# NVlabs/UnseenObjectClustering

Hardware: AMD Instinct MI355X
Metric: frames/sec at 640x480 RGB-D, two-stage clustering (higher is better)
Workload: dtype f32; 1 GPU; configs[3] frames: full two-stage (crop-and-refine) segmentation of single 640x480 RGB-D frames; throughput schedule 3 streams x 4-frame launch sets (one frame at a time: `latency`); frame=640x480, seeds=100, iters=10, crop=224, total_frames=513, frames_per_gpu=513, collective=False, frames_in_flight_per_gpu=12, streams_per_gpu=3, frames_per_launch=4

## Files before the change

include/uoc_hip.h:

```cpp
#ifndef UOC_HIP_H
#define UOC_HIP_H

#include <stddef.h>
#include <stdint.h>

#ifdef __cplusplus
extern "C" {
#endif

#define UOC_OK 0
#define UOC_EINVAL (-22)
#define UOC_ENOMEM (-12)
#define UOC_EHIP (-5)
#define UOC_ENOENT (-2)
#define UOC_ETIMEDOUT (-110)

#define UOC_EMBED_DIM 64
#define UOC_MAX_SEEDS 128
#define UOC_METRIC_COSINE 0
#define UOC_METRIC_EUCLIDEAN 1

int uoc_version(void);
int uoc_is_dev_build(void);
unsigned long long uoc_config_fingerprint(void);
int uoc_shutdown(void);
const char *uoc_last_error(void);
int uoc_reload_env(void);


int uoc_ms_set_persistent_fps(int on);
int uoc_ms_set_stream_ordering(int on);
int uoc_ms_fps_fallbacks(void);
int uoc_ms_check(void *stream);

size_t uoc_ms_workspace_bytes(int batch, int n, int m);

int uoc_ms_select_seeds(const float *d_X, int batch, int n, int m, const int32_t *d_first_index,
                        float *d_seeds, int32_t *d_indices, void *d_ws, size_t ws_bytes, void *stream);

int uoc_ms_select_seeds_from(const float *d_X, int batch, int n, int m, int num_init, const int32_t *d_first_index,
                             float *d_seeds, int32_t *d_indices, void *d_ws, size_t ws_bytes, void *stream);

int uoc_ms_hill_climb(const float *d_X, int batch, int n, float *d_Z, int m, float kappa, int iters,
                      void *d_ws, size_t ws_bytes, void *stream);

int uoc_ms_seed_components(const float *d_Z, int batch, int m, float epsilon, int32_t *d_seed_labels,
                           int32_t *d_num_unique, void *stream);

int uoc_ms_assign(const float *d_X, int batch, int n, const float *d_Z, const int32_t *d_seed_labels,
                  const int32_t *d_num_unique, int m, int32_t *d_labels, int32_t *d_closest,
                  void *d_ws, size_t ws_bytes, void *stream);

int uoc_ms_cluster(const float *d_X, int batch, int n, int m, float kappa, int iters, float epsilon,
                   const int32_t *d_first_index, int32_t *d_labels, int32_t *d_indices,
                   float *d_Z_out, int32_t *d_seed_labels_out, void *d_ws, size_t ws_bytes, void *stream);

size_t uoc_ms_workspace_bytes_wide(int batch, int n, int m, int halves);
int uoc_ms_cluster_wide(const float *d_X, int halves, int batch, int n, int m, float kappa, int iters, float epsilon,
                        const int32_t *d_first_index, int32_t *d_labels, int32_t *d_indices, float *d_Z_out,
                        int32_t *d_seed_labels_out, void *d_ws, size_t ws_bytes, void *stream);

int uoc_ms_select_seeds_ex(const float *d_X, int batch, int n, int m, int num_init, const int32_t *d_first_index,
                           float *d_seeds, int32_t *d_indices, int metric, void *d_ws, size_t ws_bytes, void *stream);
int uoc_ms_hill_climb_ex(const float *d_X, int batch, int n, float *d_Z, int m, float kappa, int iters, int metric,
                         void *d_ws, size_t ws_bytes, void *stream);
int uoc_ms_seed_components_ex(const float *d_Z, int batch, int m, float epsilon, int metric, int32_t *d_seed_labels,
                              int32_t *d_num_unique, void *stream);
int uoc_ms_assign_ex(const float *d_X, int batch, int n, const float *d_Z, const int32_t *d_seed_labels,
                     const int32_t *d_num_unique, int m, int metric, int32_t *d_labels, int32_t *d_closest, void *d_ws,
                     size_t ws_bytes, void *stream);
int uoc_ms_cluster_ex(const float *d_X, int batch, int n, int m, float kappa, int iters, float epsilon, int metric,
                      const int32_t *d_first_index, int32_t *d_labels, int32_t *d_indices, float *d_Z_out,
                      int32_t *d_seed_labels_out, void *d_ws, size_t ws_bytes, void *stream);
int uoc_ms_cluster_wide_ex(const float *d_X, int halves, int batch, int n, int m, float kappa, int iters, float epsilon,
                           int metric, const int32_t *d_first_index, int32_t *d_labels, int32_t *d_indices, float *d_Z_out,
                           int32_t *d_seed_labels_out, void *d_ws, size_t ws_bytes, void *stream);


typedef struct uoc_net uoc_net;

enum { UOC_NET_RGBD_ADD = 0, UOC_NET_COLOR = 1, UOC_NET_DEPTH = 2, UOC_NET_RGBD_EARLY = 3, UOC_NET_RGBD_CAT = 4 };

int uoc_net_create(uoc_net **out);
int uoc_net_create_mode(uoc_net **out, int mode);
int uoc_net_embed_dim(const uoc_net *net);
int uoc_net_destroy(uoc_net *net);
int uoc_net_load_param(uoc_net *net, const char *name, const float *host_data, size_t numel);
int uoc_net_finalize(uoc_net *net);
size_t uoc_net_workspace_bytes(const uoc_net *net, int B, int H, int W);
int uoc_net_set_split_precision(uoc_net *net, int on);
int uoc_net_forward(uoc_net *net, const float *d_rgb, const float *d_xyz, int B, int H, int W, float *d_embed,
                    void *d_ws, size_t ws_bytes, void *stream);

#define UOC_CONV_DIRECT 0
#define UOC_CONV_WINOGRAD4 4
#define UOC_CONV_WINOGRAD4_BF16X3 5
int uoc_conv2d_nhwc(const float *d_in, const float *d_w, const float *d_bias, const float *d_res, float *d_out,
                    int G, int B, int H, int W, int Cin, int Cout, int K, int stride, int dil, int pad, int relu,
                    void *stream);
int uoc_conv2d_nhwc_algo(const float *d_in, const float *d_w, const float *d_bias, const float *d_res, float *d_out,
                         int G, int B, int H, int W, int Cin, int Cout, int K, int stride, int dil, int pad, int relu,
                         int algo, void *stream);

int uoc_conv2d_tile_list(int algo, int32_t *out_pairs, int cap);
int uoc_conv2d_nhwc_tile(const float *d_in, const float *d_w, const float *d_bias, const float *d_res, float *d_out,
                         int G, int B, int H, int W, int Cin, int Cout, int K, int stride, int dil, int pad, int relu,
                         int algo, void *stream, int cfg, int bm);
int uoc_conv2d_tile_choice(int G, int B, int H, int W, int Cin, int Cout, int K, int stride, int dil, int algo,
                           int32_t *cfg, int32_t *bm, int32_t *family_bm);
int uoc_net_stem(const float *d_nchw, const float *h_w, const float *h_bias, const float *d_res, int G, int B, int H,
                 int W, int relu, float *d_out, void *stream);
int uoc_maxpool3x3s2_nhwc(const float *d_in, float *d_out, int n_img, int H, int W, int C, void *stream);
int uoc_head(const float *d_fa, const float *d_fb, float *d_embed, int B, int h, int w, int H, int W, int cat,
             void *stream);


typedef struct uoc_roi_table {
  int32_t K;
  int32_t label[128];
  int32_t box[128][4];
} uoc_roi_table;

size_t uoc_roi_workspace_bytes(void);

int uoc_prep_rgbd(const uint8_t *d_bgr, const uint16_t *d_depth_mm, int H, int W, float fx, float fy, float px,
                  float py, float mean_b, float mean_g, float mean_r, float *d_image, float *d_xyz, void *stream);

int uoc_filter_labels_depth(int32_t *d_labels, const float *d_z, long z_batch_stride, int B, int H, int W,
                            float threshold, void *d_ws, size_t ws_bytes, void *stream);

int uoc_roi_build(int32_t *d_labels, const float *d_z, int H, int W, float threshold, float pad_fraction,
                  uoc_roi_table *d_table, void *d_ws, size_t ws_bytes, void *stream);

int uoc_roi_crop(const float *d_rgb, const float *d_xyz, const int32_t *d_labels, int H, int W,
                 const uoc_roi_table *d_table, int K, int S, float *d_rgb_crops, float *d_xyz_crops,
                 float *d_mask_crops, void *stream);

int uoc_roi_match_stats(const int32_t *d_labels_crop, const float *d_mask_crops, const float *d_xyz_crops, int K,
                        int S, int32_t *d_keep, float *d_meanz, void *d_ws, size_t ws_bytes, void *stream);

int uoc_roi_paste(const int32_t *d_labels_crop, const uoc_roi_table *d_table, const int32_t *d_map,
                  const int32_t *d_order, int K, int S, int H, int W, int32_t *d_refined, void *stream);

int uoc_roi_match(const int32_t *d_labels_crop, const float *d_mask_crops, const float *d_xyz_crops,
                  const uoc_roi_table *d_table, int K, int S, int H, int W, int32_t *d_refined, int32_t *d_keep,
                  int32_t *d_plan, int32_t *d_status, void *d_ws, size_t ws_bytes, void *stream);

int uoc_labels_to_u8(const int32_t *d_labels, long n, uint8_t *d_out, int32_t *d_top, void *stream);


typedef struct uoc_eval_tables {
  int32_t cont[128 * 128];
  int32_t prec_tp[128 * 128];
  int32_t rec_tp[128 * 128];
  int32_t bnd_pred[128];
  int32_t bnd_gt[128];
  int32_t bad_label;
} uoc_eval_tables;

size_t uoc_eval_workspace_bytes(int H, int W);
int uoc_eval_pair_stats(const int32_t *d_pred, const int32_t *d_gt, int H, int W, int radius, uoc_eval_tables *d_tables,
                        void *d_ws, size_t ws_bytes, void *stream);


#define UOC_OBJECTS_MAX_ATTR 8
typedef struct uoc_object {
  int32_t pixels;
  int32_t count;
  int32_t box[4];
  float centroid[3];
  float cov[6];
  float aabb_min[3];
  float aabb_max[3];
  float eig[3];
  float axes[9];
  float obb_center[3];
  float obb_half[3];
  int32_t offset;
  int32_t kept;
} uoc_object;

size_t uoc_objects_workspace_bytes(int B, int H, int W);
int uoc_objects(const int32_t *d_labels, const float *d_xyz, const float *d_attr, int attr_ch, int B, int H, int W,
                int max_points_per_object, uoc_object *d_objects, float *d_points, float *d_point_attr,
                int32_t *d_point_pixel, long capacity, int32_t *d_total, void *d_ws, size_t ws_bytes, void *stream);


typedef struct uoc_track {
  int32_t uid;
  int32_t age;
  int32_t hits;
  int32_t area;
  int32_t born;
} uoc_track;
#define UOC_TRACK_SLOTS 128
#define UOC_TRACK_HEADER_WORDS 1024
#define UOC_TRACK_META_WORD 640
#define UOC_TRACK_CONT_WORDS (128 * 128)

size_t uoc_track_state_bytes(int B, int H, int W);
size_t uoc_track_workspace_bytes(int B);
int uoc_track_reset(void *d_state, int B, int H, int W, int which, void *stream);
int uoc_track_step(const int32_t *d_labels, int B, int H, int W, int q, int max_age, void *d_state, int32_t *d_out,
                   int32_t *d_lut, uoc_track *d_tracks, void *d_ws, size_t ws_bytes, void *stream);


#define UOC_CC_ALL 0
#define UOC_CC_LARGEST 1

size_t uoc_cc_workspace_bytes(int B, int H, int W);
int uoc_cc_split(const int32_t *d_labels, int B, int H, int W, int connectivity, int min_area, int mode, int32_t *d_out,
                 int32_t *d_table, int32_t *d_counts, void *d_ws, size_t ws_bytes, void *stream);


typedef struct uoc_plane {
  int32_t found;
  int32_t candidates;
  int32_t inliers;
  int32_t hyp;
  float normal[3];
  float d;
  float centroid[3];
  float eig[3];
  float rms;
  float u[3];
  float v[3];
} uoc_plane;

typedef struct uoc_plane_object {
  int32_t count;
  float height_min;
  float height_max;
  float foot[2];
  float cov2[3];
  float axis[2];
  float half[3];
  float center[3];
} uoc_plane_object;
#define UOC_PLANE_MAX_HYP 1024
#define UOC_PLANE_MAX_TAU_MM 1000

size_t uoc_plane_workspace_bytes(int B, int H, int W, int num_hyp);
int uoc_support_plane(const int32_t *d_labels, const float *d_xyz, int B, int H, int W, int num_hyp, int tau_mm,
                      uint32_t seed, uoc_plane *d_planes, uoc_plane_object *d_objs, float *d_height, void *d_ws,
                      size_t ws_bytes, void *stream);


typedef struct uoc_plane_info {
  int32_t round_candidates;
  int32_t removed;
  float cos0;
  float offset0;
  float extent[4];
} uoc_plane_info;
#define UOC_PLANES_MAX 8
#define UOC_PLANES_FRINGE 16

size_t uoc_planes_workspace_bytes(int B, int H, int W, int num_hyp, int max_planes);
int uoc_support_planes(const int32_t *d_labels, const float *d_xyz, int B, int H, int W, int max_planes, int num_hyp,
                       int tau_mm, int rem_mm, int min_inliers, uint32_t seed, int32_t *d_count, uoc_plane *d_planes,
                       uoc_plane_info *d_info, int32_t *d_index, uoc_plane_object *d_objs, void *d_ws, size_t ws_bytes,
                       void *stream);


#define UOC_REL_BORDER 0
#define UOC_REL_TOUCH 1
#define UOC_REL_FRONT 2
#define UOC_REL_MAX_GAP_MM 65535

typedef struct uoc_relation_object {
  int32_t pixels;
  int32_t edge;
  int32_t border;
  int32_t border_bg;
  int32_t hidden;
  int32_t n_touch;
  int32_t n_above;
  int32_t n_below;
  int32_t layer;
  int32_t free;
  int32_t order;
} uoc_relation_object;

size_t uoc_relations_workspace_bytes(int B, int H, int W);
int uoc_relations(const int32_t *d_labels, const float *d_xyz, int B, int H, int W, int connectivity, int gap_mm,
                  int min_pairs, int32_t *d_pairs, uoc_relation_object *d_objs, void *d_ws, size_t ws_bytes, void *stream);


#define UOC_PLACE_MAX_QUERIES 16
#define UOC_PLACE_WIDEST 0
#define UOC_PLACE_NEAREST 1
#define UOC_PLACE_MAX_GRID 512
#define UOC_PLACE_MAX_MM 1000
#define UOC_PLACE_MAX_MIN_PTS 65535
#define UOC_PLACE_MAX_ANCHOR 4096
#define UOC_PLACE_SCALE 16384

size_t uoc_placement_workspace_bytes(int B, int H, int W, int G);
int uoc_placement(const int32_t *d_labels, const float *d_xyz, const uoc_plane *d_planes, int B, int H, int W, int G,
                  int cell_mm, int h_obs_mm, int tau_mm, int min_pts, int unknown_blocks, const int32_t *h_queries, int Q,
                  int32_t *d_state, int32_t *d_owner, int32_t *d_dist2, int32_t *d_counts, int64_t *d_frame,
                  int32_t *d_answers, void *d_ws, size_t ws_bytes, void *stream);


#define UOC_GRASP_MAX_DIRS 32
#define UOC_GRASP_MISS (-1)
#define UOC_GRASP_WIDE (-2)
#define UOC_GRASP_PINCHED (-3)
#define UOC_GRASP_BLOCKED (-4)
#define UOC_GRASP_SCALE 16384
#define UOC_GRASP_MAX_OFFSETS 8
#define UOC_GRASP_MAX_OPEN 64
#define UOC_GRASP_MAX_GAP 4
#define UOC_GRASP_MAX_FINGER 8
#define UOC_GRASP_MAX_PAD 4

size_t uoc_grasp_workspace_bytes(int B, int G, int A, int M);
int uoc_grasp(const int32_t *d_state, const int32_t *d_owner, int B, int G, const int32_t *h_dirs, int A, int M, int Wmax,
              int gap, int F, int Hp, int unknown_blocks, int32_t *d_cand, int32_t *d_best, void *d_ws, size_t ws_bytes,
              void *stream);


#define UOC_ELEV_MAX_QUERIES 16
#define UOC_ELEV_NONE (-32768)

size_t uoc_elevation_workspace_bytes(int B, int H, int W, int G);
int uoc_elevation(const int32_t *d_labels, const float *d_xyz, const int64_t *d_frame, int B, int H, int W, int G,
                  int cell_mm, int tau_mm, int step_mm, int min_pts, const int32_t *h_queries, int Q, int32_t *d_elev,
                  int32_t *d_owner, int32_t *d_pts, int32_t *d_near, int32_t *d_dist2, int32_t *d_tops, int32_t *d_info,
                  int32_t *d_answers, void *d_ws, size_t ws_bytes, void *stream);


#define UOC_FOOT_MAX_RECTS 8
#define UOC_FOOT_MAX_HALF 16384
#define UOC_FOOT_ROOMIEST 0
#define UOC_FOOT_NEAREST 1

size_t uoc_footprint_workspace_bytes(int B, int G, int A, int F);
int uoc_footprint(const int32_t *d_state, const int32_t *d_owner, const int32_t *d_dist2, const int64_t *d_frame, int B, int G,
                  const int32_t *h_dirs, int A, const int32_t *h_rects, int F, int unknown_blocks, int32_t *d_fits,
                  int32_t *d_count, int32_t *d_best, void *d_ws, size_t ws_bytes, void *stream);


#define UOC_ROUTES_MAX_QUERIES 8
#define UOC_ROUTES_MAX_NEED2 4096
#define UOC_ROUTES_MAX_PATH 4096

size_t uoc_routes_workspace_bytes(int B, int G, int Q);
int uoc_routes(const int32_t *d_state, const int32_t *d_owner, const int64_t *d_frame, int B, int G, const int32_t *h_queries,
               int Q, int unknown_blocks, int max_path, int32_t *d_cost, int32_t *d_info, int32_t *d_path, void *d_ws,
               size_t ws_bytes, void *stream);


#define UOC_CONF_MAX_N (1 << 30)
#define UOC_CONF_ONE 65536

size_t uoc_ms_confidence_workspace_bytes(int batch, int n, int m, int halves);
int uoc_ms_confidence(const float *d_X, int halves, int batch, int n, const float *d_Z, const int32_t *d_seed_labels,
                      const int32_t *d_num_unique, int m, int metric, int32_t *d_labels, float *d_margin,
                      int32_t *d_second, int32_t *d_closest, int32_t *d_rival, void *d_ws, size_t ws_bytes, void *stream);
int uoc_conf_paste(const float *d_values_crop, const int32_t *d_labels_crop, const uoc_roi_table *d_table,
                   const int32_t *d_plan, int K, int S, int H, int W, float *d_out, void *stream);
int uoc_conf_objects(const int32_t *d_labels, const float *d_conf, int B, int H, int W, int weak_q, int64_t *d_stats,
                     void *stream);


#define UOC_NORMAL_UP 1
#define UOC_NORMAL_SIDE 2
#define UOC_NORMAL_OBLIQUE 3
#define UOC_NORMAL_DOWN 4
#define UOC_NORMALS_MAX_DIRS 32
#define UOC_NORMALS_FACE_WORDS 40

size_t uoc_normals_workspace_bytes(int B, int H, int W);
int uoc_normals(const float *d_xyz, const int32_t *d_labels, const uoc_plane *d_planes, int B, int H, int W, int step,
                int window, int jump_mm, int min_pairs, const int32_t *h_dirs, int A, int c_up, int s_side, int32_t *d_n,
                float *d_unit, int32_t *d_faces, void *d_ws, size_t ws_bytes, void *stream);


#define UOC_SIG_WORDS 104
#define UOC_SIG_MAX_N (1 << 24)
#define UOC_SIG_PIXELS 0
#define UOC_SIG_VALID 1
#define UOC_SIG_AREA 2
#define UOC_SIG_HIST 8
#define UOC_SIG_DARK 89
#define UOC_SIG_INTENSITY 90
#define UOC_IDENT_WORDS 5
#define UOC_IDENT_HEADER_WORDS 1024
#define UOC_IDENT_META_WORD 640

size_t uoc_signature_workspace_bytes(int B);
int uoc_signature(const int32_t *d_labels, const uint8_t *d_image, const float *d_xyz, int B, int H, int W, int32_t *d_sig,
                  void *d_ws, size_t ws_bytes, void *stream);
int uoc_sig_similarity(const int32_t *d_sig_a, const int32_t *d_sig_b, int B, int32_t *d_sim, void *stream);
size_t uoc_ident_state_bytes(int B);
size_t uoc_ident_workspace_bytes(int B);
int uoc_ident_reset(void *d_state, int B, int which, void *stream);
int uoc_ident_step(const int32_t *d_tracked, const uoc_track *d_tracks, const int32_t *d_sig, int B, int H, int W, int q, int r,
                   int max_lost, void *d_state, int32_t *d_out, int32_t *d_lut, int32_t *d_ident, void *d_ws, size_t ws_bytes,
                   void *stream);

#define UOC_MOTION_MAX_ROT 64
#define UOC_MOTION_MAX_RADIUS 16
#define UOC_MOTION_MAX_PAIRS 16
#define UOC_MOTION_MAX_CELLS 4096
#define UOC_MOTION_SCALE 16384
#define UOC_MOTION_ROT_WORDS 4
#define UOC_MOTION_BEST_WORDS 16

size_t uoc_motion_workspace_bytes(int B, int G, int A, int P);
int uoc_motion(const int32_t *d_state_a, const int32_t *d_owner_a, const int64_t *d_frame_a, const int32_t *d_state_b,
               const int32_t *d_owner_b, const int64_t *d_frame_b, int B, int G, const int32_t *h_rot, int A, int R,
               const int32_t *h_pairs, int P, int32_t *d_rot, int32_t *d_best, void *d_ws, size_t ws_bytes, void *stream);

#define UOC_SCENE_META_WORD 32
#define UOC_SCENE_MEM_WORD 48
#define UOC_SCENE_MAX_AGE 32767
#define UOC_SCENE_ID_WORDS 8
#define UOC_SCENE_INFO_WORDS 8
#define UOC_SCENE_SAME 0
#define UOC_SCENE_APPEARED 1
#define UOC_SCENE_VANISHED 2
#define UOC_SCENE_REOWNED 3

size_t uoc_scene_state_bytes(int B, int G);
size_t uoc_scene_workspace_bytes(int B, int G);
int uoc_scene_reset(void *d_state, int B, int G, int which, void *stream);
int uoc_scene_step(const int32_t *d_state_cur, const int32_t *d_owner_cur, const int64_t *d_frame, const int32_t *d_drop,
                   int B, int G, int max_age, int unknown_blocks, const int32_t *h_queries, int Q, void *d_mem,
                   int32_t *d_state, int32_t *d_owner, int32_t *d_dist2, int32_t *d_age, int32_t *d_change,
                   int32_t *d_ids, int32_t *d_info, int32_t *d_answers, void *d_ws, size_t ws_bytes, void *stream);


long uoc_lzf_decompress(const uint8_t *in, size_t in_len, uint8_t *out, size_t out_cap);

int uoc_prof_enable(int on);
int uoc_prof_reset(void);
int uoc_prof_report(char *buf, size_t cap);

#ifdef __cplusplus
static_assert(sizeof(uoc_roi_table) == 2564, "uoc_roi_table");
static_assert(sizeof(uoc_object) == 164, "uoc_object");
static_assert(sizeof(uoc_track) == 20, "uoc_track");
static_assert(sizeof(uoc_plane) == 84, "uoc_plane");
static_assert(sizeof(uoc_plane_object) == 64, "uoc_plane_object");
static_assert(sizeof(uoc_plane_info) == 32, "uoc_plane_info");
static_assert(sizeof(uoc_relation_object) == 44, "uoc_relation_object");
#endif

#ifdef __cplusplus
}
#endif
#endif
```

unseenobjectclustering_amd/_native.py:

```python
from __future__ import annotations

import ctypes
import os
from ctypes import c_char_p, c_float, c_int, c_int32, c_long, c_size_t, c_uint32, c_ulonglong, c_void_p, POINTER

from .build import LIB_PATH

_lib = None


class NativeError(RuntimeError):
    pass


P, I, F, Z, L, U = c_void_p, c_int, c_float, c_size_t, c_long, c_uint32
ABI = {
    "uoc_version": (I, []),
    "uoc_is_dev_build": (I, []),
    "uoc_config_fingerprint": (c_ulonglong, []),
    "uoc_shutdown": (I, []),
    "uoc_last_error": (c_char_p, []),
    "uoc_reload_env": (I, []),
    "uoc_ms_set_persistent_fps": (I, [I]),
    "uoc_ms_set_stream_ordering": (I, [I]),
    "uoc_ms_fps_fallbacks": (I, []),
    "uoc_ms_check": (I, [P]),
    "uoc_ms_workspace_bytes": (Z, [I, I, I]),
    "uoc_ms_select_seeds": (I, [P, I, I, I, P, P, P, P, Z, P]),
    "uoc_ms_select_seeds_from": (I, [P, I, I, I, I, P, P, P, P, Z, P]),
    "uoc_ms_hill_climb": (I, [P, I, I, P, I, F, I, P, Z, P]),
    "uoc_ms_seed_components": (I, [P, I, I, F, P, P, P]),
    "uoc_ms_assign": (I, [P, I, I, P, P, P, I, P, P, P, Z, P]),
    "uoc_ms_cluster": (I, [P, I, I, I, F, I, F, P, P, P, P, P, P, Z, P]),
    "uoc_ms_workspace_bytes_wide": (Z, [I, I, I, I]),
    "uoc_ms_cluster_wide": (I, [P, I, I, I, I, F, I, F, P, P, P, P, P, P, Z, P]),
    "uoc_ms_select_seeds_ex": (I, [P, I, I, I, I, P, P, P, I, P, Z, P]),
    "uoc_ms_hill_climb_ex": (I, [P, I, I, P, I, F, I, I, P, Z, P]),
    "uoc_ms_seed_components_ex": (I, [P, I, I, F, I, P, P, P]),
    "uoc_ms_assign_ex": (I, [P, I, I, P, P, P, I, I, P, P, P, Z, P]),
    "uoc_ms_cluster_ex": (I, [P, I, I, I, F, I, F, I, P, P, P, P, P, P, Z, P]),
    "uoc_ms_cluster_wide_ex": (I, [P, I, I, I, I, F, I, F, I, P, P, P, P, P, P, Z, P]),
    "uoc_net_create": (I, [POINTER(P)]),
    "uoc_net_create_mode": (I, [POINTER(P), I]),
    "uoc_net_embed_dim": (I, [P]),
    "uoc_net_destroy": (I, [P]),
    "uoc_net_load_param": (I, [P, c_char_p, P, Z]),
    "uoc_net_finalize": (I, [P]),
    "uoc_net_workspace_bytes": (Z, [P, I, I, I]),
    "uoc_net_set_split_precision": (I, [P, I]),
    "uoc_net_forward": (I, [P, P, P, I, I, I, P, P, Z, P]),
    "uoc_conv2d_nhwc": (I, [P, P, P, P, P, I, I, I, I, I, I, I, I, I, I, I, P]),
    "uoc_conv2d_nhwc_algo": (I, [P, P, P, P, P, I, I, I, I, I, I, I, I, I, I, I, I, P]),
    "uoc_conv2d_tile_list": (I, [I, P, I]),
    "uoc_conv2d_nhwc_tile": (I, [P, P, P, P, P, I, I, I, I, I, I, I, I, I, I, I, I, P, I, I]),
    "uoc_conv2d_tile_choice": (I, [I, I, I, I, I, I, I, I, I, I, P, P, P]),
    "uoc_net_stem": (I, [P, P, P, P, I, I, I, I, I, P, P]),
    "uoc_maxpool3x3s2_nhwc": (I, [P, P, I, I, I, I, P]),
    "uoc_head": (I, [P, P, P, I, I, I, I, I, I, P]),
    "uoc_roi_workspace_bytes": (Z, []),
    "uoc_prep_rgbd": (I, [P, P, I, I, F, F, F, F, F, F, F, P, P, P]),
    "uoc_filter_labels_depth": (I, [P, P, L, I, I, I, F, P, Z, P]),
    "uoc_roi_build": (I, [P, P, I, I, F, F, P, P, Z, P]),
    "uoc_roi_crop": (I, [P, P, P, I, I, P, I, I, P, P, P, P]),
    "uoc_roi_match_stats": (I, [P, P, P, I, I, P, P, P, Z, P]),
    "uoc_roi_paste": (I, [P, P, P, P, I, I, I, I, P, P]),
    "uoc_roi_match": (I, [P, P, P, P, I, I, I, I, P, P, P, P, P, Z, P]),
    "uoc_labels_to_u8": (I, [P, L, P, P, P]),
    "uoc_eval_workspace_bytes": (Z, [I, I]),
    "uoc_eval_pair_stats": (I, [P, P, I, I, I, P, P, Z, P]),
    "uoc_objects_workspace_bytes": (Z, [I, I, I]),
    "uoc_objects": (I, [P, P, P, I, I, I, I, I, P, P, P, P, L, P, P, Z, P]),
    "uoc_track_state_bytes": (Z, [I, I, I]),
    "uoc_track_workspace_bytes": (Z, [I]),
    "uoc_track_reset": (I, [P, I, I, I, I, P]),
    "uoc_track_step": (I, [P, I, I, I, I, I, P, P, P, P, P, Z, P]),
    "uoc_cc_workspace_bytes": (Z, [I, I, I]),
    "uoc_cc_split": (I, [P, I, I, I, I, I, I, P, P, P, P, Z, P]),
    "uoc_plane_workspace_bytes": (Z, [I, I, I, I]),
    "uoc_support_plane": (I, [P, P, I, I, I, I, I, U, P, P, P, P, Z, P]),
    "uoc_planes_workspace_bytes": (Z, [I, I, I, I, I]),
    "uoc_support_planes": (I, [P, P, I, I, I, I, I, I, I, I, U, P, P, P, P, P, P, Z, P]),
    "uoc_relations_workspace_bytes": (Z, [I, I, I]),
    "uoc_relations": (I, [P, P, I, I, I, I, I, I, P, P, P, Z, P]),
    "uoc_placement_workspace_bytes": (Z, [I, I, I, I]),
    "uoc_placement": (I, [P, P, P, I, I, I, I, I, I, I, I, I, P, I, P, P, P, P, P, P, P, Z, P]),
    "uoc_grasp_workspace_bytes": (Z, [I, I, I, I]),
    "uoc_grasp": (I, [P, P, I, I, P, I, I, I, I, I, I, I, P, P, P, Z, P]),
    "uoc_elevation_workspace_bytes": (Z, [I, I, I, I]),
    "uoc_elevation": (I, [P, P, P, I, I, I, I, I, I, I, I, P, I, P, P, P, P, P, P, P, P, P, Z, P]),
    "uoc_footprint_workspace_bytes": (Z, [I, I, I, I]),
    "uoc_footprint": (I, [P, P, P, P, I, I, P, I, P, I, I, P, P, P, P, Z, P]),
    "uoc_routes_workspace_bytes": (Z, [I, I, I]),
    "uoc_routes": (I, [P, P, P, I, I, P, I, I, I, P, P, P, P, Z, P]),
    "uoc_ms_confidence_workspace_bytes": (Z, [I, I, I, I]),
    "uoc_ms_confidence": (I, [P, I, I, I, P, P, P, I, I, P, P, P, P, P, P, Z, P]),
    "uoc_conf_paste": (I, [P, P, P, P, I, I, I, I, P, P]),
    "uoc_conf_objects": (I, [P, P, I, I, I, I, P, P]),
    "uoc_normals_workspace_bytes": (Z, [I, I, I]),
    "uoc_normals": (I, [P, P, P, I, I, I, I, I, I, I, P, I, I, I, P, P, P, P, Z, P]),
    "uoc_signature_workspace_bytes": (Z, [I]),
    "uoc_signature": (I, [P, P, P, I, I, I, P, P, Z, P]),
    "uoc_sig_similarity": (I, [P, P, I, P, P]),
    "uoc_ident_state_bytes": (Z, [I]),
    "uoc_ident_workspace_bytes": (Z, [I]),
    "uoc_ident_reset": (I, [P, I, I, P]),
    "uoc_ident_step": (I, [P, P, P, I, I, I, I, I, I, P, P, P, P, P, Z, P]),
    "uoc_motion_workspace_bytes": (Z, [I, I, I, I]),
    "uoc_motion": (I, [P, P, P, P, P, P, I, I, P, I, I, P, I, P, P, P, Z, P]),
    "uoc_scene_state_bytes": (Z, [I, I]),
    "uoc_scene_workspace_bytes": (Z, [I, I]),
    "uoc_scene_reset": (I, [P, I, I, I, P]),
    "uoc_scene_step": (I, [P, P, P, P, I, I, I, I, P, I, P, P, P, P, P, P, P, P, P, P, Z, P]),
    "uoc_lzf_decompress": (L, [P, Z, P, Z]),
    "uoc_prof_enable": (I, [I]),
    "uoc_prof_reset": (I, []),
    "uoc_prof_report": (I, [c_char_p, Z]),
}
EXPORTED_SYMBOLS = tuple(ABI)


def _declare(lib):
    for name, (restype, argtypes) in ABI.items():
        fn = getattr(lib, name)
        fn.restype, fn.argtypes = restype, argtypes


METRIC_COSINE = 0
METRIC_EUCLIDEAN = 1
METRICS = {"cosine": METRIC_COSINE, "euclidean": METRIC_EUCLIDEAN}
METRIC_SYMBOLS = ("uoc_ms_select_seeds_ex", "uoc_ms_hill_climb_ex", "uoc_ms_seed_components_ex", "uoc_ms_assign_ex",
                  "uoc_ms_cluster_ex", "uoc_ms_cluster_wide_ex")


TILE_SYMBOLS = ("uoc_conv2d_tile_list", "uoc_conv2d_nhwc_tile", "uoc_conv2d_tile_choice", "uoc_net_stem",
                "uoc_maxpool3x3s2_nhwc", "uoc_head")


def metric_code(metric) -> int:
    if metric not in METRICS:
        raise NotImplementedError(f"metric={metric!r}: only 'cosine' and 'euclidean' are implemented on gfx950")
    return METRICS[metric]


class RoiTable(ctypes.Structure):
    _fields_ = [("K", c_int32), ("label", c_int32 * 128), ("box", (c_int32 * 4) * 128)]


ROI_TABLE_BYTES = ctypes.sizeof(RoiTable)


class UocObject(ctypes.Structure):
    _fields_ = [("pixels", c_int32), ("count", c_int32), ("box", c_int32 * 4), ("centroid", c_float * 3), ("cov", c_float * 6),
                ("aabb_min", c_float * 3), ("aabb_max", c_float * 3), ("eig", c_float * 3), ("axes", c_float * 9),
                ("obb_center", c_float * 3), ("obb_half", c_float * 3), ("offset", c_int32), ("kept", c_int32)]


OBJECT_BYTES = ctypes.sizeof(UocObject)


class UocPlane(ctypes.Structure):
    _fields_ = [("found", c_int32), ("candidates", c_int32), ("inliers", c_int32), ("hyp", c_int32), ("normal", c_float * 3),
                ("d", c_float), ("centroid", c_float * 3), ("eig", c_float * 3), ("rms", c_float), ("u", c_float * 3),
                ("v", c_float * 3)]


class UocPlaneObject(ctypes.Structure):
    _fields_ = [("count", c_int32), ("height_min", c_float), ("height_max", c_float), ("foot", c_float * 2),
                ("cov2", c_float * 3), ("axis", c_float * 2), ("half", c_float * 3), ("center", c_float * 3)]


class UocPlaneInfo(ctypes.Structure):
    _fields_ = [("round_candidates", c_int32), ("removed", c_int32), ("cos0", c_float), ("offset0", c_float),
                ("extent", c_float * 4)]


class UocRelationObject(ctypes.Structure):
    _fields_ = [(name, c_int32) for name in ("pixels", "edge", "border", "border_bg", "hidden", "n_touch", "n_above", "n_below",
                                             "layer", "free", "order")]


REL_BORDER, REL_TOUCH, REL_FRONT = 0, 1, 2
REL_MAX_GAP_MM = 65535
PLANE_MAX_HYP = 1024
PLANE_MAX_TAU_MM = 1000
PLANES_MAX = 8
PLANES_FRINGE = 16
PLACE_WIDEST, PLACE_NEAREST = 0, 1
PLACE_MAX_QUERIES = 16
PLACE_MAX_GRID = 512
PLACE_MAX_MM = 1000
PLACE_MAX_MIN_PTS = 65535
PLACE_MAX_ANCHOR = 4096
PLACE_SCALE = 16384
GRASP_MISS, GRASP_WIDE, GRASP_PINCHED, GRASP_BLOCKED = -1, -2, -3, -4
GRASP_SCALE = 16384
GRASP_MAX_DIRS = 32
GRASP_MAX_OFFSETS = 8
GRASP_MAX_OPEN = 64
GRASP_MAX_GAP = 4
GRASP_MAX_FINGER = 8
GRASP_MAX_PAD = 4
ELEV_NONE = -32768
ELEV_MAX_QUERIES = 16
FOOT_MAX_RECTS = 8
FOOT_MAX_HALF = 16384
FOOT_ROOMIEST, FOOT_NEAREST = 0, 1
ROUTES_MAX_QUERIES = 8
ROUTES_MAX_NEED2 = 4096
ROUTES_MAX_PATH = 4096
CONF_MAX_N = 1 << 30
CONF_ONE = 65536
NORMAL_UP, NORMAL_SIDE, NORMAL_OBLIQUE, NORMAL_DOWN = 1, 2, 3, 4
NORMALS_MAX_DIRS = 32
NORMALS_FACE_WORDS = 40
SIG_WORDS = 104
SIG_MAX_N = 1 << 24
SIG_PIXELS, SIG_VALID, SIG_AREA, SIG_HIST, SIG_DARK, SIG_INTENSITY = 0, 1, 2, 8, 89, 90
IDENT_WORDS = 5
IDENT_HEADER_WORDS = 1024
IDENT_META_WORD = 640
IDENT_FIELDS = ("pid", "uid", "seen", "hits", "pixels")
MOTION_MAX_ROT = 64
MOTION_MAX_RADIUS = 16
MOTION_MAX_PAIRS = 16
MOTION_MAX_CELLS = 4096
MOTION_SCALE = 16384
MOTION_ROT_WORDS, MOTION_BEST_WORDS = 4, 16
SCENE_META_WORD, SCENE_MEM_WORD = 32, 48
SCENE_MAX_AGE = 32767
SCENE_ID_WORDS, SCENE_INFO_WORDS = 8, 8
SCENE_SAME, SCENE_APPEARED, SCENE_VANISHED, SCENE_REOWNED = 0, 1, 2, 3


class UocTrack(ctypes.Structure):
    _fields_ = [("uid", c_int32), ("age", c_int32), ("hits", c_int32), ("area", c_int32), ("born", c_int32)]


TRACK_FIELDS = tuple(name for name, _ in UocTrack._fields_)
TRACK_SLOTS = 128
TRACK_HEADER_WORDS = 1024
TRACK_META_WORD = 640
TRACK_CONT_WORDS = 128 * 128
CC_ALL, CC_LARGEST = 0, 1
CC_MODES = {"all": CC_ALL, "largest": CC_LARGEST}
CC_FIELDS = ("src", "area", "root", "siblings")
OBJECTS_MAX_ATTR = 8


def lib():
    global _lib
    if _lib is None:
        if not os.path.exists(LIB_PATH):
            raise NativeError(
                f"{LIB_PATH} not found: build it with `python -m unseenobjectclustering_amd.build` "
                "(or __graft_entry__.build()).  There is no CPU fallback.")
        import torch
        l = ctypes.CDLL(LIB_PATH)
        try:
            _declare(l)
        except AttributeError as e:
            raise NativeError(f"{LIB_PATH} lacks a symbol of include/uoc_hip.h ({e}): rebuild it with "
                              "`python -m unseenobjectclustering_amd.build`") from e
        _lib = l
        import atexit
        atexit.register(l.uoc_shutdown)
    return _lib


CONV_DIRECT, CONV_WINOGRAD4, CONV_WINOGRAD4_BF16X3 = 0, 4, 5


def config_fingerprint() -> int:
    return int(lib().uoc_config_fingerprint())


def check(rc: int, what: str):
    if rc != 0:
        msg = lib().uoc_last_error().decode("utf-8", "replace")
        raise NativeError(f"{what} failed (rc={rc}): {msg}")


def on_gpu(t) -> bool:
    import torch
    return isinstance(t, torch.Tensor) and t.device.type == "cuda"


class Fields:

    def __init__(self, **fields):
        self.__dict__.update(fields)


def as_labels(labels):
    import torch
    return (labels if labels.dtype == torch.int32 else labels.to(torch.int32)).contiguous()


def label_input(who, labels):
    if not on_gpu(labels):
        raise NativeError(f"{who}: labels must be a tensor on the GPU (there is no CPU fallback)")
    return as_labels(labels)


def frame_inputs(who, labels, xyz):
    import torch
    for t, what in ((labels, "labels"), (xyz, "xyz")):
        if not on_gpu(t):
            raise NativeError(f"{who}: {what} must be a tensor on the GPU (there is no CPU fallback)")
    if labels.dim() == 2:
        labels = labels[None]
    if xyz.dim() == 3:
        xyz = xyz[None]
    if labels.dim() != 3 or xyz.dim() != 4 or xyz.shape[1] != 3 or xyz.shape[0] != labels.shape[0] \
            or tuple(xyz.shape[2:]) != tuple(labels.shape[1:]):
        raise NativeError(f"{who}: labels {tuple(labels.shape)} and xyz {tuple(xyz.shape)} do not match "
                          "([B,H,W] and [B,3,H,W])")
    if xyz.device != labels.device:
        raise NativeError(f"{who}: labels and xyz are on different devices")
    return as_labels(labels), xyz.to(torch.float32).contiguous()


def grid_inputs(who, state, owner):
    for t, what in ((state, "state"), (owner, "owner")):
        if not on_gpu(t):
            raise NativeError(f"{who}: {what} must be a tensor on the GPU (there is no CPU fallback)")
    state, owner = (t[None] if t.dim() == 2 else t for t in (state, owner))
    if state.dim() != 3 or state.shape[1] != state.shape[2] or tuple(owner.shape) != tuple(state.shape) or owner.device != state.device:
        raise NativeError(f"{who}: state {tuple(state.shape)} and owner {tuple(owner.shape)} are not two [B,G,G] grids on one device")
    return as_labels(state), as_labels(owner)


def ptr(t):
    if t is None:
        return c_void_p(0)
    return c_void_p(t.data_ptr())


def stream_ptr(device=None):
    import torch
    return c_void_p(torch.cuda.current_stream(device).cuda_stream)


def call(name, device, *args, stream=True):
    import torch
    fn = getattr(lib(), name)
    args = [a.data_ptr() if hasattr(a, "data_ptr") else a for a in args]
    if device is None:
        rc = fn(*args)
    else:
        with torch.cuda.device(device):
            rc = fn(*args, torch.cuda.current_stream(device).cuda_stream) if stream else fn(*args)
    check(rc, name)


def workspace(name, device, *shape, who, hint):
    import torch
    nbytes = getattr(lib(), name)(*shape)
    if nbytes == 0:
        raise NativeError(f"{who}: bad shape {hint}")
    return torch.empty(nbytes, dtype=torch.uint8, device=device)


def host_words(rows, width):
    flat = [int(x) for row in rows for x in row]
    return (c_int32 * max(len(flat), width))(*flat)


def stream_key(device):
    import torch
    index = torch.cuda.current_device() if device.index is None else device.index
    return (device.type, index, int(torch.cuda.current_stream(device).cuda_stream))


_retired = []
GRAPHS_ALIVE = 0


def retire(t):
    if t is not None and GRAPHS_ALIVE > 0:
        _retired.append(t)


class PerStream:

    def __init__(self, make, size=None):
        self.make, self.size, self.items = make, size, {}

    def get(self, device, need=0):
        key = stream_key(device)
        obj = self.items.get(key)
        if obj is None or (self.size is not None and self.size(obj) < need):
            retire(obj)
            obj = self.items[key] = self.make(device, need)
        return obj

    def of_device(self, device):
        where = stream_key(device)[:2]
        return [obj for key, obj in self.items.items() if key[:2] == where]


def prof_enable(on: bool):
    lib().uoc_prof_reset()
    lib().uoc_prof_enable(1 if on else 0)


def prof_report():
    import json
    buf = ctypes.create_string_buffer(1 << 19)
    call("uoc_prof_report", None, buf, len(buf))
    return json.loads(buf.value.decode())
```

unseenobjectclustering_amd/csrc/conv.h:

```cpp
#pragma once
#include "common.h"

namespace uoc {

struct ConvParams {
  const float *in;
  const float *w;
  const float *bias;
  const float *res;
  float *out;
  int G, B, H, W, Cin, Ho, Wo, Cout;
  int KH, KW, stride, dil, pad, relu;
  int stem;
  int tune = 1;
  int prof_kc = -1;
  double prof_flops = 0.0;
  int prof_tag[4] = {0, 0, 0, 0};
};

int launch_conv(const ConvParams &p, hipStream_t st);
int conv_tile_list(int *out_pairs, int cap);
int conv_tile_choice(const ConvParams &p, int *cfg, int *bm, int *fam_bm);
int launch_conv_tile(const ConvParams &p, hipStream_t st, int cfg, int bm);

struct W4Tile {
  int bm, bn;
};
int wino4_tile_list(bool split, int *out_pairs, int cap);
void wino4_tile_choice(bool split, int NT, int Cout, int planes, int *bn, int *bm);
int wino4_split_tile_list(int *out_pairs, int cap);
void wino4_split_tile_choice(int NT, int Cout, int planes, int *bn, int *bm);
void wino4_pick_tile(const int (*tiles)[2], int n, int NT, int Cout, int planes, int &bm, int &bn);
int wino4_plane_grid(int NT, int Cout, int planes, int bm, int bn);

bool wino4_eligible(const ConvParams &p);
bool wino4_channels_ok(int Cin, int Cout);
size_t wino4_ws_floats(int G, int B, int H, int W, int d, int Cin, int Cout);
int wino4_num_tiles(int B, int H, int W, int d);
int launch_wino4_weights(const float *w, float *U, int G, int Cout, int Cin, hipStream_t st);
int launch_wino4_conv(const ConvParams &p, const float *U, float *ws, hipStream_t st, const unsigned short *U3 = nullptr,
                      const W4Tile *tile = nullptr);
int launch_wino4_split_weights(const float *U, unsigned short *U3, int G, int Cout, int Cin, hipStream_t st);
int launch_wino4_slice_split(const ConvParams &p0, int Bg, int b0, const unsigned short *U3, float *ws, hipStream_t st,
                             const W4Tile *tile = nullptr);
struct Wino4Geom;
int w4_stage_output(const ConvParams &p, const Wino4Geom &geo, const float *Mw, hipStream_t st);
long wino4_elem_blocks(long items);
int launch_nchw3_to_nhwc4(const float *in, float *out, int B, int H, int W, hipStream_t st);
int launch_maxpool3x3s2(const float *in, float *out, int n_img, int H, int W, int C, int Ho, int Wo, hipStream_t st);
int launch_head(const float *fa, const float *fb, float *embed, int B, int h, int w, int H, int W, int cat,
                hipStream_t st);

}
```

unseenobjectclustering_amd/csrc/net.hip:

```cpp
#include <map>
#include <mutex>
#include <string>
#include <vector>

#include "conv.h"

#include <stdlib.h>

namespace uoc {

struct ConvLayer {
  std::string conv, bn;
  int Cin, Cout, K, stride, dil, pad, relu;
  bool has_bn, has_bias, stem;
  float *d_w = nullptr, *d_b = nullptr;
  float *d_U4 = nullptr;
  unsigned short *d_U3 = nullptr;
  size_t w_per_group = 0;
};

struct Block {
  int conv1, conv2, down;
};

}

struct uoc_net {
  std::map<std::string, std::vector<float>> params;
  std::vector<uoc::ConvLayer> layers;
  std::vector<uoc::Block> blocks;
  int stem = -1, fc = -1;
  bool finalized = false;
  int device = -1;
  const int wino_min_cin = 64;
  const int wino_f = 4;
  bool split = false;
  int mode = UOC_NET_RGBD_ADD;
  int G = 2;
};

namespace uoc {

static const char *kBranch[2] = {"fcn", "fcn_depth"};

static int add_conv(uoc_net *n, const std::string &conv, const std::string &bn, int Cin, int Cout, int K, int stride,
                    int dil, int relu, bool has_bn, bool has_bias, bool stem = false) {
  ConvLayer L;
  L.conv = conv;
  L.bn = bn;
  L.Cin = Cin;
  L.Cout = Cout;
  L.K = K;
  L.stride = stride;
  L.dil = dil;
  L.pad = stem ? 3 : (K == 3 ? dil : 0);
  L.relu = relu;
  L.has_bn = has_bn;
  L.has_bias = has_bias;
  L.stem = stem;
  n->layers.push_back(L);
  return (int)n->layers.size() - 1;
}

static void build_graph(uoc_net *n) {
  n->stem = add_conv(n, "conv1", "bn1", n->mode == UOC_NET_RGBD_EARLY ? 6 : 3, 64, 7, 2, 1, 1, true, false, true);
  const int nblocks[4] = {3, 4, 6, 3};
  const int planes[4] = {64, 128, 256, 512};
  int inpl = 64, cur_stride = 4, cur_dil = 1;
  for (int li = 0; li < 4; ++li) {
    int stride = li == 0 ? 1 : 2;
    const bool need_down = stride != 1 || inpl != planes[li];
    if (need_down) {
      if (cur_stride == 8) {
        cur_dil *= stride;
        stride = 1;
      } else {
        cur_stride *= stride;
      }
    }
    for (int bi = 0; bi < nblocks[li]; ++bi) {
      const std::string pfx = "layer" + std::to_string(li + 1) + "." + std::to_string(bi) + ".";
      Block b;
      const int s = bi == 0 ? stride : 1;
      const int cin = bi == 0 ? inpl : planes[li];
      b.conv1 = add_conv(n, pfx + "conv1", pfx + "bn1", cin, planes[li], 3, s, cur_dil, 1, true, false);
      b.conv2 = add_conv(n, pfx + "conv2", pfx + "bn2", planes[li], planes[li], 3, 1, cur_dil, 1, true, false);
      b.down = -1;
      if (bi == 0 && need_down)
        b.down = add_conv(n, pfx + "downsample.0", pfx + "downsample.1", cin, planes[li], 1, s, 1, 0, true, false);
      n->blocks.push_back(b);
    }
    inpl = planes[li];
  }
  n->fc = add_conv(n, "fc", "", 512, 64, 1, 1, 1, 0, false, true);
}

static const std::vector<float> *find(const uoc_net *n, const std::string &key, size_t numel) {
  auto it = n->params.find(key);
  if (it == n->params.end()) {
    set_error("missing parameter '%s'", key.c_str());
    return nullptr;
  }
  if (it->second.size() != numel) {
    set_error("parameter '%s' has %zu elements, expected %zu", key.c_str(), it->second.size(), numel);
    return nullptr;
  }
  return &it->second;
}

static void relayout_weights(const float *w, const double *scale, int Cout, int Cin, int K, bool stem, size_t w_per_group,
                             float *dst) {
  for (int co = 0; co < Cout; ++co)
    for (int ci = 0; ci < Cin; ++ci)
      for (int kh = 0; kh < K; ++kh)
        for (int kw = 0; kw < K; ++kw) {
          const double v = (double)w[(((size_t)co * Cin + ci) * K + kh) * K + kw] * scale[co];
          size_t o;
          if (stem)
            o = (size_t)(ci / 3) * w_per_group + ((size_t)kh * Cout + co) * 32 + kw * 4 + ci % 3;
          else
            o = ((size_t)(kh * K + kw) * Cout + co) * Cin + ci;
          dst[o] = (float)v;
        }
}

static int finalize_layer(uoc_net *n, ConvLayer &L) {
  const int G = n->G;
  const int T = L.stem ? 7 : L.K * L.K;
  const int Kc = L.stem ? 32 : L.Cin;
  const int sets = L.stem ? L.Cin / 3 : 1;
  L.w_per_group = (size_t)T * L.Cout * Kc;
  std::vector<float> hw((size_t)G * sets * L.w_per_group, 0.f), hb((size_t)(G + 1) * L.Cout, 0.f);
  for (int g = 0; g < G; ++g) {
    const std::string base = std::string(kBranch[g]) + ".resnet34_8s.";
    const auto *w = find(n, base + L.conv + ".weight", (size_t)L.Cout * L.Cin * L.K * L.K);
    if (!w) return UOC_ENOENT;
    std::vector<double> scale(L.Cout, 1.0), shift(L.Cout, 0.0);
    if (L.has_bn) {
      const auto *ga = find(n, base + L.bn + ".weight", L.Cout);
      const auto *be = find(n, base + L.bn + ".bias", L.Cout);
      const auto *mu = find(n, base + L.bn + ".running_mean", L.Cout);
      const auto *va = find(n, base + L.bn + ".running_var", L.Cout);
      if (!ga || !be || !mu || !va) return UOC_ENOENT;
      for (int c = 0; c < L.Cout; ++c) {
        const double inv = 1.0 / sqrt((double)(*va)[c] + 1e-5);
        scale[c] = (double)(*ga)[c] * inv;
        shift[c] = (double)(*be)[c] - (double)(*mu)[c] * scale[c];
      }
    }
    if (L.has_bias) {
      const auto *bi = find(n, base + L.conv + ".bias", L.Cout);
      if (!bi) return UOC_ENOENT;
      for (int c = 0; c < L.Cout; ++c) shift[c] += (double)(*bi)[c];
    }
    relayout_weights(w->data(), scale.data(), L.Cout, L.Cin, L.K, L.stem, L.w_per_group,
                     hw.data() + (size_t)g * sets * L.w_per_group);
    for (int c = 0; c < L.Cout; ++c) hb[(size_t)g * L.Cout + c] = (float)shift[c];
  }
  UOC_HIP_CHECK(hipMalloc(&L.d_w, hw.size() * sizeof(float)));
  UOC_HIP_CHECK(hipMalloc(&L.d_b, hb.size() * sizeof(float)));
  UOC_HIP_CHECK(hipMemcpy(L.d_w, hw.data(), hw.size() * sizeof(float), hipMemcpyHostToDevice));
  UOC_HIP_CHECK(hipMemcpy(L.d_b, hb.data(), hb.size() * sizeof(float), hipMemcpyHostToDevice));
  if (!L.stem && L.K == 3 && L.stride == 1 && n->wino_min_cin > 0 && L.Cin >= n->wino_min_cin && L.Cin % 32 == 0 &&
      L.Cout % 64 == 0) {
    if (n->wino_f == 4 && !wino4_channels_ok(L.Cin, L.Cout)) {
    } else if (n->wino_f == 4) {
      UOC_HIP_CHECK(hipMalloc(&L.d_U4, (size_t)G * 36 * L.Cout * L.Cin * sizeof(float)));
      if (int rc = launch_wino4_weights(L.d_w, L.d_U4, G, L.Cout, L.Cin, nullptr)) return rc;
    }
    UOC_HIP_CHECK(hipDeviceSynchronize());
  }
  return UOC_OK;
}

struct Dims {
  int H1, W1, H2, W2, H3, W3;
};
static Dims dims(int H, int W) {
  Dims d;
  d.H1 = (H - 1) / 2 + 1;
  d.W1 = (W - 1) / 2 + 1;
  d.H2 = (d.H1 - 1) / 2 + 1;
  d.W2 = (d.W1 - 1) / 2 + 1;
  d.H3 = (d.H2 - 1) / 2 + 1;
  d.W3 = (d.W2 - 1) / 2 + 1;
  return d;
}

struct NetWs {
  float *in4, *stem, *stem_part, *buf[4], *fc, *wino;
  size_t total;
};
static NetWs carve_net(void *base, int mode, int wino_f, int B, int H, int W) {
  const Dims d = dims(H, W);
  const int G = (mode == UOC_NET_RGBD_ADD || mode == UOC_NET_RGBD_CAT) ? 2 : 1;
  const int n_in = (G == 2 || mode == UOC_NET_RGBD_EARLY) ? 2 : 1;
  NetWs w;
  Carver cv(base);
  w.in4 = cv.take<float>((size_t)n_in * B * H * W * 4);
  w.stem = cv.take<float>((size_t)G * B * d.H1 * d.W1 * 64);
  w.stem_part = mode == UOC_NET_RGBD_EARLY ? cv.take<float>((size_t)B * d.H1 * d.W1 * 64) : nullptr;
  size_t act = (size_t)G * B * d.H2 * d.W2 * 64;
  const size_t a3 = (size_t)G * B * d.H3 * d.W3 * 512;
  if (a3 > act) act = a3;
  for (int i = 0; i < 4; ++i) w.buf[i] = cv.take<float>(act);
  w.fc = cv.take<float>((size_t)G * B * d.H3 * d.W3 * 64);
  size_t wv = 0;
  if (wino_f == 4) {
    const int cand[6][4] = {{3, 4, 512, 512}, {3, 4, 256, 512}, {3, 2, 256, 256}, {3, 2, 128, 256}, {3, 1, 128, 128}, {2, 1, 64, 64}};
    for (const auto &c : cand) {
      const size_t v = wino4_ws_floats(G, B, c[0] == 3 ? d.H3 : d.H2, c[0] == 3 ? d.W3 : d.W2, c[1], c[2], c[3]);
      if (v > wv) wv = v;
    }
  }
  w.wino = cv.take<float>(wv);
  w.total = cv.total();
  return w;
}

static ConvParams conv_params(int G, const ConvLayer &L, const float *in, const float *res, float *out, int B, int H, int W,
                              int Ho, int Wo) {
  ConvParams p;
  p.in = in;
  p.w = L.d_w;
  p.bias = L.d_b;
  p.res = res;
  p.out = out;
  p.G = G;
  p.B = B;
  p.H = H;
  p.W = W;
  p.Cin = L.stem ? 4 : L.Cin;
  p.Ho = Ho;
  p.Wo = Wo;
  p.Cout = L.Cout;
  p.KH = p.KW = L.K;
  p.stride = L.stride;
  p.dil = L.dil;
  p.pad = L.pad;
  p.relu = L.relu;
  p.stem = L.stem ? 1 : 0;
  return p;
}

static int run_conv(int G, const ConvLayer &L, const float *in, const float *res, float *out, int B, int H, int W,
                    int Ho, int Wo, hipStream_t st, float *wino_ws = nullptr, bool split = false) {
  const ConvParams p = conv_params(G, L, in, res, out, B, H, W, Ho, Wo);
  if (L.d_U4 && wino_ws && wino4_eligible(p))
    return launch_wino4_conv(p, L.d_U4, wino_ws, st, split ? L.d_U3 : nullptr);
  return launch_conv(p, st);
}

}

using namespace uoc;

extern "C" {

int uoc_net_create(uoc_net **out) { return uoc_net_create_mode(out, UOC_NET_RGBD_ADD); }

int uoc_net_create_mode(uoc_net **out, int mode) {
  UOC_REQUIRE(out != nullptr, "out is null");
  UOC_REQUIRE(mode >= UOC_NET_RGBD_ADD && mode <= UOC_NET_RGBD_CAT, "unknown network mode %d", mode);
  uoc_net *n = new (std::nothrow) uoc_net();
  if (!n) {
    set_error("out of host memory");
    return UOC_ENOMEM;
  }
  n->mode = mode;
  n->G = (mode == UOC_NET_RGBD_ADD || mode == UOC_NET_RGBD_CAT) ? 2 : 1;
  build_graph(n);
  *out = n;
  return UOC_OK;
}

int uoc_net_set_split_precision(uoc_net *n, int on) {
  UOC_REQUIRE(n && n->finalized, "uoc_net_set_split_precision: the network must be finalized");
  if (on) {
    for (auto &L : n->layers) {
      if (!L.d_U4 || L.d_U3) continue;
      const size_t elems = (size_t)n->G * 36 * 3 * L.Cout * L.Cin;
      UOC_HIP_CHECK(hipMalloc(&L.d_U3, elems * sizeof(unsigned short)));
      if (int rc = launch_wino4_split_weights(L.d_U4, L.d_U3, n->G, L.Cout, L.Cin, nullptr)) return rc;
    }
    UOC_HIP_CHECK(hipDeviceSynchronize());
  }
  n->split = on != 0;
  return UOC_OK;
}

int uoc_net_embed_dim(const uoc_net *n) { return n && n->mode == UOC_NET_RGBD_CAT ? 128 : 64; }

int uoc_net_destroy(uoc_net *n) {
  if (!n) return UOC_OK;
  for (auto &L : n->layers) {
    if (L.d_w) (void)hipFree(L.d_w);
    if (L.d_b) (void)hipFree(L.d_b);
    if (L.d_U4) (void)hipFree(L.d_U4);
    if (L.d_U3) (void)hipFree(L.d_U3);
  }
  delete n;
  return UOC_OK;
}

int uoc_net_load_param(uoc_net *n, const char *name, const float *host, size_t numel) {
  UOC_REQUIRE(n && name && host, "null argument");
  UOC_REQUIRE(!n->finalized, "network already finalized");
  n->params[std::string(name)] = std::vector<float>(host, host + numel);
  return UOC_OK;
}

int uoc_net_finalize(uoc_net *n) {
  UOC_REQUIRE(n != nullptr, "net is null");
  UOC_REQUIRE(!n->finalized, "network already finalized");
  UOC_HIP_CHECK(hipGetDevice(&n->device));
  for (auto &L : n->layers)
    if (int rc = finalize_layer(n, L)) return rc;
  n->params.clear();
  n->finalized = true;
  return UOC_OK;
}

size_t uoc_net_workspace_bytes(const uoc_net *n, int B, int H, int W) {
  if (!n || B < 1 || H < 8 || W < 8) return 0;
  return carve_net(nullptr, n->mode, n->wino_f, B, H, W).total;
}

int uoc_net_forward(uoc_net *n, const float *d_rgb, const float *d_xyz, int B, int H, int W, float *d_embed,
                    void *d_ws, size_t ws_bytes, void *stream) {
  UOC_REQUIRE(n && n->finalized, "network not finalized");
  UOC_REQUIRE(d_embed && (d_rgb || n->mode == UOC_NET_DEPTH) && (d_xyz || n->mode == UOC_NET_COLOR),
              "null tensor pointer");
  UOC_REQUIRE(B >= 1 && H >= 8 && W >= 8, "bad input shape B=%d H=%d W=%d", B, H, W);
  const int G = n->G;
  const NetWs w = carve_net(d_ws, n->mode, n->wino_f, B, H, W);
  UOC_REQUIRE(d_ws && ws_bytes >= w.total && ((uintptr_t)d_ws & 255) == 0, "workspace too small or misaligned (%zu < %zu)",
              ws_bytes, w.total);
  hipStream_t st = (hipStream_t)stream;
  const Dims d = dims(H, W);

  const ConvLayer &stem = n->layers[n->stem];
  const size_t in_stride = (size_t)B * H * W * 4;
  if (n->mode == UOC_NET_RGBD_EARLY) {
    if (int rc = launch_nchw3_to_nhwc4(d_rgb, w.in4, B, H, W, st)) return rc;
    if (int rc = launch_nchw3_to_nhwc4(d_xyz, w.in4 + in_stride, B, H, W, st)) return rc;
    ConvLayer part = stem;
    part.d_w = stem.d_w + stem.w_per_group;
    part.d_b = stem.d_b + (size_t)G * stem.Cout;
    part.relu = 0;
    if (int rc = run_conv(1, part, w.in4 + in_stride, nullptr, w.stem_part, B, H, W, d.H1, d.W1, st)) return rc;
    if (int rc = run_conv(1, stem, w.in4, w.stem_part, w.stem, B, H, W, d.H1, d.W1, st)) return rc;
  } else {
    const float *first = n->mode == UOC_NET_DEPTH ? d_xyz : d_rgb;
    if (int rc = launch_nchw3_to_nhwc4(first, w.in4, B, H, W, st)) return rc;
    if (G == 2)
      if (int rc = launch_nchw3_to_nhwc4(d_xyz, w.in4 + in_stride, B, H, W, st)) return rc;
    if (int rc = run_conv(G, stem, w.in4, nullptr, w.stem, B, H, W, d.H1, d.W1, st)) return rc;
  }
  if (int rc = launch_maxpool3x3s2(w.stem, w.buf[0], G * B, d.H1, d.W1, 64, d.H2, d.W2, st)) return rc;

  int cur = 0, h = d.H2, wd = d.W2;
  for (const Block &b : n->blocks) {
    const ConvLayer &c1 = n->layers[b.conv1], &c2 = n->layers[b.conv2];
    const int ho = (h - 1) / c1.stride + 1, wo = (wd - 1) / c1.stride + 1;
    float *x = w.buf[cur], *tmp = w.buf[(cur + 1) & 3], *sc = w.buf[(cur + 2) & 3], *y = w.buf[(cur + 3) & 3];
    if (int rc = run_conv(G, c1, x, nullptr, tmp, B, h, wd, ho, wo, st, w.wino, n->split)) return rc;
    const float *res = x;
    if (b.down >= 0) {
      if (int rc = run_conv(G, n->layers[b.down], x, nullptr, sc, B, h, wd, ho, wo, st)) return rc;
      res = sc;
    }
    if (int rc = run_conv(G, c2, tmp, res, y, B, ho, wo, ho, wo, st, w.wino, n->split)) return rc;
    cur = (cur + 3) & 3;
    h = ho;
    wd = wo;
  }
  if (int rc = run_conv(G, n->layers[n->fc], w.buf[cur], nullptr, w.fc, B, h, wd, h, wd, st)) return rc;
  return launch_head(w.fc, G == 2 ? w.fc + (size_t)B * h * wd * 64 : nullptr, d_embed, B, h, wd, H, W,
                     n->mode == UOC_NET_RGBD_CAT, st);
}

static ConvParams entry_params(int G, int B, int H, int W, int Cin, int Cout, int K, int stride, int dil, int pad, int relu) {
  ConvParams p;
  p.tune = 0;
  p.in = p.w = p.bias = p.res = nullptr;
  p.out = nullptr;
  p.G = G;
  p.B = B;
  p.H = H;
  p.W = W;
  p.Cin = Cin;
  p.Cout = Cout;
  p.KH = p.KW = K;
  p.stride = stride;
  p.dil = dil;
  p.pad = pad;
  p.relu = relu;
  p.stem = 0;
  p.Ho = (H + 2 * pad - dil * (K - 1) - 1) / stride + 1;
  p.Wo = (W + 2 * pad - dil * (K - 1) - 1) / stride + 1;
  return p;
}

static int conv2d_entry(const float *d_in, const float *d_w, const float *d_bias, const float *d_res, float *d_out, int G,
                        int B, int H, int W, int Cin, int Cout, int K, int stride, int dil, int pad, int relu, int algo,
                        void *stream, const int *tile) {
  UOC_REQUIRE(K == 1 || K == 3, "K=%d (only 1 or 3)", K);
  UOC_REQUIRE(G >= 1 && B >= 1 && H >= 1 && W >= 1 && Cin >= 1 && Cout >= 1 && stride >= 1 && dil >= 1 && pad >= 0,
              "conv2d: bad shape");
  UOC_REQUIRE(d_res == nullptr || d_res != d_out, "conv2d: the residual must not alias the output");
  ConvParams p = entry_params(G, B, H, W, Cin, Cout, K, stride, dil, pad, relu);
  p.in = d_in;
  p.w = d_w;
  p.bias = d_bias;
  p.res = d_res;
  p.out = d_out;
  hipStream_t st = (hipStream_t)stream;
  if (algo == UOC_CONV_DIRECT) return tile ? launch_conv_tile(p, st, tile[0], tile[1]) : launch_conv(p, st);
  const W4Tile w4tile = {tile ? tile[1] : 0, tile ? tile[0] : 0};
  const W4Tile *wt = tile ? &w4tile : nullptr;
  static std::mutex mu;
  std::lock_guard<std::mutex> lock(mu);
  if (algo == UOC_CONV_WINOGRAD4 || algo == UOC_CONV_WINOGRAD4_BF16X3) {
    UOC_REQUIRE(wino4_eligible(p), "conv2d: shape not eligible for Winograd F(4x4,3x3)");
    if (tile) {
      int pairs[2 * 32];
      const int n = wino4_tile_list(algo == UOC_CONV_WINOGRAD4_BF16X3, pairs, 32);
      bool listed = false;
      for (int i = 0; i < n && i < 32; ++i) listed = listed || (pairs[2 * i] == tile[0] && pairs[2 * i + 1] == tile[1]);
      UOC_REQUIRE(listed, "conv2d tile: the plane GEMM has no tile BN=%d BM=%d", tile[0], tile[1]);
      UOC_REQUIRE(Cout % tile[0] == 0, "conv2d tile: Cout=%d is not a multiple of BN=%d", Cout, tile[0]);
    }
    static float *U4 = nullptr, *ws4 = nullptr;
    static unsigned short *U3 = nullptr;
    static size_t ucap4 = 0, wcap4 = 0, ucap3 = 0;
    const size_t un = (size_t)G * 36 * Cout * Cin, wn = wino4_ws_floats(G, B, H, W, dil, Cin, Cout);
    if (un > ucap4) {
      if (U4) (void)hipFree(U4);
      UOC_HIP_CHECK(hipMalloc(&U4, un * sizeof(float)));
      ucap4 = un;
    }
    if (wn > wcap4) {
      if (ws4) (void)hipFree(ws4);
      UOC_HIP_CHECK(hipMalloc(&ws4, wn * sizeof(float)));
      wcap4 = wn;
    }
    if (int rc = launch_wino4_weights(d_w, U4, G, Cout, Cin, st)) return rc;
    if (algo == UOC_CONV_WINOGRAD4_BF16X3) {
      if (3 * un > ucap3) {
        if (U3) (void)hipFree(U3);
        UOC_HIP_CHECK(hipMalloc(&U3, 3 * un * sizeof(unsigned short)));
        ucap3 = 3 * un;
      }
      if (int rc = launch_wino4_split_weights(U4, U3, G, Cout, Cin, st)) return rc;
      return launch_wino4_conv(p, U4, ws4, st, U3, wt);
    }
    return launch_wino4_conv(p, U4, ws4, st, nullptr, wt);
  }
  set_error("conv2d: unknown algorithm %d", algo);
  return UOC_EINVAL;
}

int uoc_conv2d_nhwc_algo(const float *d_in, const float *d_w, const float *d_bias, const float *d_res, float *d_out, int G,
                         int B, int H, int W, int Cin, int Cout, int K, int stride, int dil, int pad, int relu, int algo,
                         void *stream) {
  return conv2d_entry(d_in, d_w, d_bias, d_res, d_out, G, B, H, W, Cin, Cout, K, stride, dil, pad, relu, algo, stream, nullptr);
}

int uoc_conv2d_nhwc_tile(const float *d_in, const float *d_w, const float *d_bias, const float *d_res, float *d_out, int G,
                         int B, int H, int W, int Cin, int Cout, int K, int stride, int dil, int pad, int relu, int algo,
                         void *stream, int cfg, int bm) {
  UOC_REQUIRE(d_in && d_w && d_out, "conv2d tile: null pointer");
  const int tile[2] = {cfg, bm};
  return conv2d_entry(d_in, d_w, d_bias, d_res, d_out, G, B, H, W, Cin, Cout, K, stride, dil, pad, relu, algo, stream, tile);
}

int uoc_conv2d_tile_list(int algo, int32_t *out_pairs, int cap) {
  UOC_REQUIRE(cap >= 0 && (out_pairs || cap == 0), "tile list: null array");
  if (algo == UOC_CONV_DIRECT) return conv_tile_list(out_pairs, cap);
  if (algo == UOC_CONV_WINOGRAD4 || algo == UOC_CONV_WINOGRAD4_BF16X3)
    return wino4_tile_list(algo == UOC_CONV_WINOGRAD4_BF16X3, out_pairs, cap);
  set_error("tile list: unknown algorithm %d", algo);
  return UOC_EINVAL;
}

int uoc_conv2d_tile_choice(int G, int B, int H, int W, int Cin, int Cout, int K, int stride, int dil, int algo, int32_t *cfg,
                           int32_t *bm, int32_t *family_bm) {
  UOC_REQUIRE(cfg && bm, "tile choice: null pointer");
  UOC_REQUIRE(K == 1 || K == 3, "K=%d (only 1 or 3)", K);
  UOC_REQUIRE(G >= 1 && B >= 1 && H >= 1 && W >= 1 && Cin >= 1 && Cout >= 1 && stride >= 1 && dil >= 1, "tile choice: bad shape");
  const ConvParams p = entry_params(G, B, H, W, Cin, Cout, K, stride, dil, K == 3 ? dil : 0, 0);
  if (algo == UOC_CONV_DIRECT) return conv_tile_choice(p, cfg, bm, family_bm);
  if (algo == UOC_CONV_WINOGRAD4 || algo == UOC_CONV_WINOGRAD4_BF16X3) {
    UOC_REQUIRE(wino4_eligible(p), "tile choice: shape not eligible for Winograd F(4x4,3x3)");
    int bn_ = 0, bm_ = 0;
    wino4_tile_choice(algo == UOC_CONV_WINOGRAD4_BF16X3, wino4_num_tiles(B, H, W, dil), Cout, 36 * G, &bn_, &bm_);
    *cfg = bn_;
    *bm = bm_;
    return UOC_OK;
  }
  set_error("tile choice: unknown algorithm %d", algo);
  return UOC_EINVAL;
}

int uoc_net_stem(const float *d_nchw, const float *h_w, const float *h_bias, const float *d_res, int G, int B, int H, int W,
                 int relu, float *d_out, void *stream) {
  UOC_REQUIRE(d_nchw && h_w && d_out, "stem: null pointer");
  UOC_REQUIRE(G >= 1 && B >= 1 && H >= 1 && W >= 1, "stem: bad shape");
  UOC_REQUIRE(d_res == nullptr || d_res != d_out, "stem: the residual must not alias the output");
  UOC_REQUIRE((long)G * B * H * W * 4 < (1l << 31), "stem: input too large");
  hipStream_t st = (hipStream_t)stream;
  const size_t wpg = (size_t)7 * 64 * 32;
  std::vector<float> hw((size_t)G * wpg, 0.f), hb((size_t)G * 64, 0.f);
  const std::vector<double> one(64, 1.0);
  for (int g = 0; g < G; ++g) relayout_weights(h_w + (size_t)g * 64 * 3 * 49, one.data(), 64, 3, 7, true, wpg, hw.data() + g * wpg);
  if (h_bias) hb.assign(h_bias, h_bias + (size_t)G * 64);
  float *d_w = nullptr, *d_b = nullptr, *d_in4 = nullptr;
  int rc = UOC_OK;
  auto run = [&]() -> int {
    UOC_HIP_CHECK(hipMalloc(&d_w, hw.size() * sizeof(float)));
    UOC_HIP_CHECK(hipMalloc(&d_b, hb.size() * sizeof(float)));
    UOC_HIP_CHECK(hipMalloc(&d_in4, (size_t)G * B * H * W * 4 * sizeof(float)));
    UOC_HIP_CHECK(hipMemcpyAsync(d_w, hw.data(), hw.size() * sizeof(float), hipMemcpyHostToDevice, st));
    UOC_HIP_CHECK(hipMemcpyAsync(d_b, hb.data(), hb.size() * sizeof(float), hipMemcpyHostToDevice, st));
    if (int r = launch_nchw3_to_nhwc4(d_nchw, d_in4, G * B, H, W, st)) return r;
    ConvLayer L;
    L.Cin = 3;
    L.Cout = 64;
    L.K = 7;
    L.stride = 2;
    L.dil = 1;
    L.pad = 3;
    L.relu = relu;
    L.has_bn = L.has_bias = false;
    L.stem = true;
    L.d_w = d_w;
    L.d_b = d_b;
    const Dims d = dims(H, W);
    if (int r = run_conv(G, L, d_in4, d_res, d_out, B, H, W, d.H1, d.W1, st)) return r;
    UOC_HIP_CHECK(hipStreamSynchronize(st));
    return UOC_OK;
  };
  rc = run();
  if (rc != UOC_OK) (void)hipStreamSynchronize(st);
  if (d_w) (void)hipFree(d_w);
  if (d_b) (void)hipFree(d_b);
  if (d_in4) (void)hipFree(d_in4);
  return rc;
}

int uoc_maxpool3x3s2_nhwc(const float *d_in, float *d_out, int n_img, int H, int W, int C, void *stream) {
  UOC_REQUIRE(d_in && d_out && d_in != d_out, "maxpool: null or aliasing pointer");
  UOC_REQUIRE(n_img >= 1 && H >= 1 && W >= 1 && C >= 4, "maxpool: bad shape");
  UOC_REQUIRE((long)n_img * H * W * C < (1l << 31), "maxpool: tensor too large for 32-bit indexing");
  return launch_maxpool3x3s2(d_in, d_out, n_img, H, W, C, (H - 1) / 2 + 1, (W - 1) / 2 + 1, (hipStream_t)stream);
}

int uoc_head(const float *d_fa, const float *d_fb, float *d_embed, int B, int h, int w, int H, int W, int cat, void *stream) {
  UOC_REQUIRE(d_fa && d_embed && (d_fb || !cat), "head: null pointer");
  UOC_REQUIRE(B >= 1 && h >= 1 && w >= 1 && H >= 1 && W >= 1, "head: bad shape");
  UOC_REQUIRE((long)B * h * w * 64 < (1l << 31) && (long)B * H * W < (1l << 31) / 128, "head: tensor too large");
  return launch_head(d_fa, d_fb, d_embed, B, h, w, H, W, cat, (hipStream_t)stream);
}

int uoc_conv2d_nhwc(const float *d_in, const float *d_w, const float *d_bias, const float *d_res, float *d_out, int G,
                    int B, int H, int W, int Cin, int Cout, int K, int stride, int dil, int pad, int relu,
                    void *stream) {
  return uoc_conv2d_nhwc_algo(d_in, d_w, d_bias, d_res, d_out, G, B, H, W, Cin, Cout, K, stride, dil, pad, relu,
                              UOC_CONV_DIRECT, stream);
}

}
```

unseenobjectclustering_amd/csrc/wino4.hip:

```cpp
#include "conv.h"
#include "dma.h"
#include "prof.h"
#include "wino4_math.h"

#include <stdlib.h>

namespace uoc {

constexpr int W4BK = 32;
#ifndef W4_OUT_MIN_BLOCKS
#define W4_OUT_MIN_BLOCKS 2
#endif

__global__ __launch_bounds__(256) void wino4_weight_kernel(const float *__restrict__ w, float *__restrict__ U, int G,
                                                           int Cout, int Cin) {
  const long total = (long)G * Cout * Cin;
  for (long i = (long)blockIdx.x * blockDim.x + threadIdx.x; i < total; i += (long)gridDim.x * blockDim.x) {
    const int ci = (int)(i % Cin);
    const int co = (int)((i / Cin) % Cout);
    const int g = (int)(i / ((long)Cin * Cout));
    wino4_weight_body(w, U, G, Cout, Cin, g, co, ci);
  }
}

template <int VEC>
__global__ __launch_bounds__(256) void wino4_input_kernel(const float *__restrict__ in, float *__restrict__ V,
                                                          Wino4Geom geo, int G, int C) {
  const int CV = C / VEC;
  const long total = (long)G * geo.NT * CV;
#ifndef W4_IN_XCD
#define W4_IN_XCD 1
#endif
  const long vblock = W4_IN_XCD ? (long)(blockIdx.x & 7) * (gridDim.x >> 3) + (blockIdx.x >> 3) : (long)blockIdx.x;
  for (long idx = vblock * blockDim.x + threadIdx.x; idx < total; idx += (long)gridDim.x * blockDim.x) {
    const int cv = (int)(idx % CV);
    const int tau = (int)((idx / CV) % geo.NT);
    const int g = (int)(idx / ((long)CV * geo.NT));
    wino4_input_body<VEC>(in, V, geo, C, g, tau, cv);
  }
}

template <int VEC>
__global__ __launch_bounds__(256, W4_OUT_MIN_BLOCKS) void wino4_output_kernel(const float *__restrict__ M, const float *__restrict__ bias,
                                                           const float *__restrict__ res, float *__restrict__ out,
                                                           Wino4Geom geo, int G, int Cout, int relu) {
  const int CV = Cout / VEC;
  const long total = (long)G * geo.NT * CV;
  for (long idx = (long)blockIdx.x * blockDim.x + threadIdx.x; idx < total; idx += (long)gridDim.x * blockDim.x) {
    const int cv = (int)(idx % CV);
    const int tau = (int)((idx / CV) % geo.NT);
    const int g = (int)(idx / ((long)CV * geo.NT));
    wino4_output_body<VEC>(M, bias, res, out, geo, Cout, relu, g, tau, cv);
  }
}



__device__ __forceinline__ f32x4 w4mfma(float a, float b, f32x4 c) {
  return __builtin_amdgcn_mfma_f32_16x16x4f32(a, b, c, 0, 0, 0);
}

#ifndef UOC_W4_ABLATE
#define UOC_W4_ABLATE 0
#endif
#define W4_BARRIER() do { if (UOC_W4_ABLATE != 1) __builtin_amdgcn_s_barrier(); } while (0)
template <int N>
__device__ __forceinline__ void w4_wait_vmcnt() {
  if (UOC_W4_ABLATE != 2) wait_vmcnt<N>();
}

template <int BM, int BN, bool PAIR, int NW>
__global__ __launch_bounds__(NW * 64) void wino4_gemm_kernel(const float *__restrict__ V, const float *__restrict__ U,
                                                             float *__restrict__ Mo, int NT, int Cin, int Cout, int planes,
                                                             int mtiles, int nt_shift) {
  static_assert(NW == 8 || NW == 4, "waves per block");
  constexpr int WAVES_N = NW / 2;
  constexpr int WM = BM / 2, WN = BN / WAVES_N;
  constexpr int TM = WM / 16, TN = WN / 16;
  constexpr int R = BM + BN;
  constexpr int RPP = NW * 8;
  constexpr int NPA = (BM + RPP - 1) / RPP, NPW = (BN + RPP - 1) / RPP, NPASS = NPA + NPW;
  constexpr int STAGE = R * W4BK;
  static_assert(WM % 16 == 0 && WN % 16 == 0 && R % 8 == 0 && NPASS <= 12, "tile shape");

  extern __shared__ __attribute__((aligned(16))) float smem[];

  const int ntiles = 1 << nt_shift;
  const int per_plane = mtiles << nt_shift;
  const int total = planes * per_plane;
  const int S = (total + 7) >> 3;
  const int xcd = blockIdx.x & 7, jloc = blockIdx.x >> 3, nbl = gridDim.x >> 3;
  const int slice_lo = xcd * S, slice_hi = min(total, slice_lo + S);
  const int first = slice_lo + jloc;
  if (first >= slice_hi) return;
  const int n_items = (slice_hi - first + nbl - 1) / nbl;
  const int cpt = Cin / W4BK;
  const int nchunks = n_items * cpt;

  const unsigned lds_base = (unsigned)(size_t)((__attribute__((address_space(3))) char *)smem);
  const int tid = threadIdx.x, lane = tid & 63;
  const int wave = __builtin_amdgcn_readfirstlane(tid >> 6);
  const int wm = wave / WAVES_N, wn = wave % WAVES_N;
  const int t = lane & 15, q = lane >> 4;

  const unsigned plane_a_bytes = (unsigned)((size_t)NT * Cin * 4), plane_w_bytes = (unsigned)((size_t)Cout * Cin * 4);
  const v4i srd_a = make_srd(V, (unsigned)planes * plane_a_bytes);
  const v4i srd_w = make_srd(U, (unsigned)planes * plane_w_bytes);

  int l_r0[NPASS], l_row[NPASS], l_c4[NPASS];
#pragma unroll
  for (int j = 0; j < NPASS; ++j) {
    const bool isw = j >= NPA;
    int r0 = (isw ? BM + (j - NPA) * RPP : j * RPP) + wave * 8;
    if (!isw && r0 >= BM) r0 = BM - 8;
    if (isw && r0 >= R) r0 = R - 8;
    l_r0[j] = r0;
    const int r = r0 + (lane >> 3);
    l_row[j] = isw ? r - BM : r;
    l_c4[j] = 4 * ((lane & 7) ^ ((r >> 1) & 7));
  }

  int iss_plane, iss_rem, iss_cc = 0;
  {
    iss_plane = first / per_plane;
    iss_rem = first - iss_plane * per_plane;
  }
  unsigned l_voff[NPASS];
  unsigned soff_a, soff_w;
#define W4_ITEM_SETUP()                                                                                  \
  {                                                                                                      \
    const int mt_ = iss_rem >> nt_shift, nt_ = iss_rem & (ntiles - 1);                                   \
    _Pragma("unroll") for (int j = 0; j < NPASS; ++j) {                                                  \
      if (j < NPA) {                                                                                     \
        const int tau_ = min(mt_ * BM + l_row[j], NT - 1);                                               \
        l_voff[j] = (unsigned)((tau_ * Cin + l_c4[j]) * 4);                                              \
      } else {                                                                                           \
        l_voff[j] = (unsigned)(((nt_ * BN + l_row[j]) * Cin + l_c4[j]) * 4);                             \
      }                                                                                                  \
    }                                                                                                    \
    soff_a = (unsigned)__builtin_amdgcn_readfirstlane((int)((unsigned)iss_plane * plane_a_bytes));       \
    soff_w = (unsigned)__builtin_amdgcn_readfirstlane((int)((unsigned)iss_plane * plane_w_bytes));       \
  }
#define W4_ISSUE(STG)                                                                                    \
  {                                                                                                      \
    _Pragma("unroll") for (int j = 0; j < NPASS; ++j) {                                                  \
      const unsigned dst_ = lds_base + (unsigned)(((STG)*STAGE + l_r0[j] * W4BK) * sizeof(float));       \
      if (UOC_W4_ABLATE == 4) continue;                                                                  \
      if (j < NPA)                                                                                       \
        blds16(srd_a, l_voff[j], soff_a, dst_);                                                          \
      else                                                                                               \
        blds16(srd_w, l_voff[j], soff_w, dst_);                                                          \
    }                                                                                                    \
  }
#define W4_ADVANCE()                                                                                     \
  {                                                                                                      \
    if (++iss_cc == cpt) {                                                                               \
      iss_cc = 0;                                                                                        \
      iss_rem += nbl;                                                                                    \
      while (iss_rem >= per_plane) {                                                                     \
        iss_rem -= per_plane;                                                                            \
        ++iss_plane;                                                                                     \
      }                                                                                                  \
      W4_ITEM_SETUP()                                                                                    \
    } else {                                                                                             \
      soff_a += W4BK * 4;                                                                                \
      soff_w += W4BK * 4;                                                                                \
    }                                                                                                    \
  }
#define W4_FRAG(STG, HH, WA, XB)                                                                         \
  {                                                                                                      \
    const float *base_ = smem + (STG)*STAGE;                                                             \
    const int slot_ = ((4 * (HH) + q) ^ ((t >> 1) & 7)) * 4;                                             \
    _Pragma("unroll") for (int j = 0; j < TN; ++j) WA[j] =                                               \
        *reinterpret_cast<const float4 *>(base_ + (BM + wn * WN + 16 * j + t) * W4BK + slot_);           \
    _Pragma("unroll") for (int i = 0; i < TM; ++i) XB[i] =                                               \
        *reinterpret_cast<const float4 *>(base_ + (wm * WM + 16 * i + t) * W4BK + slot_);                \
  }
#define W4_MFMA_E(WA, XB, E)                                                                                   \
  {                                                                                                            \
    _Pragma("unroll") for (int j = 0; j < TN; ++j) _Pragma("unroll") for (int i = 0; i < TM; ++i) acc[j][i] =  \
        w4mfma(WA[j].E, XB[i].E, acc[j][i]);                                                                   \
  }

  f32x4 acc[TN][TM];
#pragma unroll
  for (int j = 0; j < TN; ++j)
#pragma unroll
    for (int i = 0; i < TM; ++i) acc[j][i] = f32x4{0.f, 0.f, 0.f, 0.f};

  int cmp_plane = iss_plane, cmp_rem = iss_rem, cmp_cc = 0;

  float4 wa0[TN], xb0[TM], wa1[TN], xb1[TM];
  const bool early = NW == 4 || wave < 4;
  auto epilogue = [&]() {
    cmp_cc = 0;
    const int mt = cmp_rem >> nt_shift, nt = cmp_rem & (ntiles - 1);
    float *dst = Mo + (size_t)cmp_plane * NT * Cout;
#pragma unroll
    for (int j = 0; j < TN; ++j) {
      const int co = nt * BN + wn * WN + 16 * j + 4 * q;
#pragma unroll
      for (int i = 0; i < TM; ++i) {
        const int m = mt * BM + wm * WM + 16 * i + t;
        if (m < NT)
          *reinterpret_cast<float4 *>(dst + (size_t)m * Cout + co) =
              make_float4(acc[j][i][0], acc[j][i][1], acc[j][i][2], acc[j][i][3]);
        acc[j][i] = f32x4{0.f, 0.f, 0.f, 0.f};
      }
    }
    cmp_rem += nbl;
    while (cmp_rem >= per_plane) {
      cmp_rem -= per_plane;
      ++cmp_plane;
    }
  };
  if constexpr (PAIR) {
    W4_ITEM_SETUP()
    W4_ISSUE(0)
    W4_ADVANCE()
    W4_ISSUE(1)
    W4_ADVANCE()
    w4_wait_vmcnt<0>();
    W4_BARRIER();
    W4_FRAG(0, 0, wa0, xb0)
    if (NW == 8 && wave >= 4) __builtin_amdgcn_s_setprio(1);
    for (int kc = 0; kc < nchunks; kc += 2) {
      const int sa = (kc & 2), sb = sa + 1, sc = sa ^ 2, sd = sc + 1;
      const bool more = kc + 2 < nchunks;
      if (more && early) {
        W4_ISSUE(sc)
        W4_ADVANCE()
        W4_ISSUE(sd)
        W4_ADVANCE()
      }
      W4_MFMA_E(wa0, xb0, x)
      W4_FRAG(sa, 1, wa1, xb1)
      __builtin_amdgcn_sched_barrier(0);
      W4_MFMA_E(wa0, xb0, y)
      W4_MFMA_E(wa0, xb0, z)
      W4_MFMA_E(wa0, xb0, w)
      if (more && !early) {
        W4_ISSUE(sc)
        W4_ADVANCE()
        W4_ISSUE(sd)
        W4_ADVANCE()
      }
      W4_FRAG(sb, 0, wa0, xb0)
      __builtin_amdgcn_sched_barrier(0);
      W4_MFMA_E(wa1, xb1, x)
      W4_MFMA_E(wa1, xb1, y)
      W4_MFMA_E(wa1, xb1, z)
      W4_MFMA_E(wa1, xb1, w)
      __builtin_amdgcn_sched_barrier(0);
      W4_MFMA_E(wa0, xb0, x)
      W4_FRAG(sb, 1, wa1, xb1)
      __builtin_amdgcn_sched_barrier(0);
      W4_MFMA_E(wa0, xb0, y)
      W4_MFMA_E(wa0, xb0, z)
      W4_MFMA_E(wa0, xb0, w)
      if (more) {
        w4_wait_vmcnt<0>();
        __builtin_amdgcn_s_waitcnt(0xC07F);
        W4_BARRIER();
        W4_FRAG(sc, 0, wa0, xb0)
      }
      __builtin_amdgcn_sched_barrier(0);
      W4_MFMA_E(wa1, xb1, x)
      W4_MFMA_E(wa1, xb1, y)
      W4_MFMA_E(wa1, xb1, z)
      W4_MFMA_E(wa1, xb1, w)
      __builtin_amdgcn_sched_barrier(0);
      __builtin_amdgcn_s_waitcnt(0xC07F);
      __builtin_amdgcn_sched_barrier(0);
      cmp_cc += 2;
      if (cmp_cc == cpt) epilogue();
    }
    return;
  }
  W4_ITEM_SETUP()
  W4_ISSUE(0)
  W4_ADVANCE()
  if (nchunks > 1) {
    W4_ISSUE(1)
    W4_ADVANCE()
    w4_wait_vmcnt<NPASS>();
  } else {
    w4_wait_vmcnt<0>();
  }
  W4_BARRIER();
  W4_FRAG(0, 0, wa0, xb0)
  int s_cur = 0, s_nxt = 1, s_nn = 2;
  if (NW == 8 && wave >= 4) __builtin_amdgcn_s_setprio(1);
  for (int kc = 0; kc < nchunks; ++kc) {
    if (kc + 2 < nchunks && early) W4_ISSUE(s_nn)
    W4_MFMA_E(wa0, xb0, x)
    W4_FRAG(s_cur, 1, wa1, xb1)
    __builtin_amdgcn_sched_barrier(0);
    W4_MFMA_E(wa0, xb0, y)
    W4_MFMA_E(wa0, xb0, z)
    W4_MFMA_E(wa0, xb0, w)
    if (kc + 2 < nchunks && !early) W4_ISSUE(s_nn)
    if (kc + 2 < nchunks) W4_ADVANCE()
    if (kc + 2 < nchunks)
      w4_wait_vmcnt<NPASS>();
    else
      w4_wait_vmcnt<0>();
    __builtin_amdgcn_s_waitcnt(0xC07F);
    W4_BARRIER();
    if (kc + 1 < nchunks) W4_FRAG(s_nxt, 0, wa0, xb0)
    __builtin_amdgcn_sched_barrier(0);
    W4_MFMA_E(wa1, xb1, x)
    W4_MFMA_E(wa1, xb1, y)
    W4_MFMA_E(wa1, xb1, z)
    W4_MFMA_E(wa1, xb1, w)
    __builtin_amdgcn_sched_barrier(0);
    __builtin_amdgcn_s_waitcnt(0xC07F);
    __builtin_amdgcn_sched_barrier(0);
    if (++cmp_cc == cpt) epilogue();
    const int tmp = s_cur;
    s_cur = s_nxt;
    s_nxt = s_nn;
    s_nn = tmp;
  }
#undef W4_ITEM_SETUP
#undef W4_ISSUE
#undef W4_ADVANCE
#undef W4_FRAG
#undef W4_MFMA_E
}

template <int BM, int BN, bool PAIR, int NW>
static int launch_wino4_gemm_t(const float *V, const float *U, float *Mo, int NT, int Cin, int Cout, int planes, int nblocks,
                               hipStream_t st) {
  const int mtiles = (NT + BM - 1) / BM, ntiles = Cout / BN;
  int nt_shift = 0;
  while ((1 << nt_shift) < ntiles) ++nt_shift;
  UOC_REQUIRE((1 << nt_shift) == ntiles, "winograd F(4x4): Cout / %d = %d is not a power of two", BN, ntiles);
  constexpr int NSTAGE = PAIR ? 4 : 3;
  const size_t lds = (size_t)NSTAGE * (BM + BN) * W4BK * sizeof(float);
  static_assert((size_t)NSTAGE * (BM + BN) * W4BK * sizeof(float) <= 160 * 1024, "LDS ring too large");
  UOC_REQUIRE(!PAIR || (Cin / W4BK) % 2 == 0, "winograd F(4x4): the pair loop needs an even number of 32-channel chunks");
  static DeviceOnce attr_set;
  if (int rc = opt_in_dynamic_lds(reinterpret_cast<const void *>(&wino4_gemm_kernel<BM, BN, PAIR, NW>), lds, attr_set)) return rc;
  hipLaunchKernelGGL((wino4_gemm_kernel<BM, BN, PAIR, NW>), dim3(nblocks), dim3(NW * 64), lds, st, V, U, Mo, NT, Cin, Cout, planes,
                     mtiles, nt_shift);
  UOC_LAUNCH_CHECK();
  return UOC_OK;
}

#define UOC_W4_TILES(X) \
  X(96, 128) X(128, 128) X(160, 128) X(192, 128) X(96, 64) X(128, 64) X(160, 64) X(192, 64)
static const int kW4Tiles[][2] = {
#define X(A, B) {A, B},
    UOC_W4_TILES(X)
#undef X
};

static int plane_per_xcd() {
  const int dev = device_num_cu(), ncu = dev > 0 ? dev : 256;
  return ncu / 8 > 0 ? ncu / 8 : 1;
}

void wino4_pick_tile(const int (*tiles)[2], int n, int NT, int Cout, int planes, int &bm, int &bn) {
  const int per_xcd = plane_per_xcd();
  double best = -1;
  for (int i = 0; i < n; ++i) {
    const int BM = tiles[i][0], BN = tiles[i][1];
    if (Cout % BN) continue;
    const long items = (long)planes * ((NT + BM - 1) / BM) * (Cout / BN);
    const long S = (items + 7) / 8;
    const long steps = (S + per_xcd - 1) / per_xcd;
    const double cost = (double)steps * BM * BN * (1.0 + 0.05 * (192.0 / BM - 1.0)) * (BN == 64 ? 1.06 : 1.0);
    if (best < 0 || cost < best) {
      best = cost;
      bm = BM;
      bn = BN;
    }
  }
}

int wino4_plane_grid(int NT, int Cout, int planes, int bm, int bn) {
  const int per_xcd = plane_per_xcd();
  const long items = (long)planes * ((NT + bm - 1) / bm) * (Cout / bn);
  const long S = (items + 7) / 8;
  return 8 * (int)(S < per_xcd ? S : per_xcd);
}

static int launch_wino4_gemm(const float *V, const float *U, float *Mo, int NT, int Cin, int Cout, int planes, hipStream_t st,
                             const W4Tile *tile) {
  int bm = 160, bn = Cout % 128 == 0 ? 128 : 64;
  if (tile) {
    bm = tile->bm;
    bn = tile->bn;
    UOC_REQUIRE((bn == 64 || bn == 128) && Cout % bn == 0, "winograd F(4x4): Cout=%d does not admit BN=%d", Cout, bn);
  } else {
    wino4_pick_tile(kW4Tiles, (int)(sizeof(kW4Tiles) / sizeof(kW4Tiles[0])), NT, Cout, planes, bm, bn);
  }
  const int nblocks = wino4_plane_grid(NT, Cout, planes, bm, bn);
  const int cpt = Cin / W4BK;
  const bool pair = cpt % 2 == 0 && cpt >= 4;
#define X(A, B)                                                                                                      \
  if (bm == A && bn == B)                                                                                            \
    return pair ? launch_wino4_gemm_t<A, B, true, 8>(V, U, Mo, NT, Cin, Cout, planes, nblocks, st)                    \
                : launch_wino4_gemm_t<A, B, false, 8>(V, U, Mo, NT, Cin, Cout, planes, nblocks, st);
  UOC_W4_TILES(X)
#undef X
  set_error("winograd F(4x4): no GEMM tile %dx%d", bm, bn);
  return UOC_EINVAL;
}

int wino4_tile_list(bool split, int *out_pairs, int cap) {
  if (split) return wino4_split_tile_list(out_pairs, cap);
  const int n = (int)(sizeof(kW4Tiles) / sizeof(kW4Tiles[0]));
  for (int i = 0; i < n && i < cap && out_pairs; ++i) {
    out_pairs[2 * i] = kW4Tiles[i][1];
    out_pairs[2 * i + 1] = kW4Tiles[i][0];
  }
  return n;
}

void wino4_tile_choice(bool split, int NT, int Cout, int planes, int *bn, int *bm) {
  if (split) return wino4_split_tile_choice(NT, Cout, planes, bn, bm);
  *bm = 160;
  *bn = Cout % 128 == 0 ? 128 : 64;
  wino4_pick_tile(kW4Tiles, (int)(sizeof(kW4Tiles) / sizeof(kW4Tiles[0])), NT, Cout, planes, *bm, *bn);
}

bool wino4_channels_ok(int Cin, int Cout) {
  const int n64 = Cout / 64;
  return Cin % W4BK == 0 && Cout % 64 == 0 && n64 > 0 && (n64 & (n64 - 1)) == 0;
}

bool wino4_eligible(const ConvParams &p) {
  return !p.stem && p.KH == 3 && p.KW == 3 && p.stride == 1 && p.pad == p.dil && wino4_channels_ok(p.Cin, p.Cout) &&
         p.Ho == p.H && p.Wo == p.W;
}

int wino4_num_tiles(int B, int H, int W, int d) { return make_geom4(B, H, W, d).NT; }

size_t wino4_ws_floats(int G, int B, int H, int W, int d, int Cin, int Cout) {
  const Wino4Geom geo = make_geom4(B, H, W, d);
  return (size_t)G * 36 * geo.NT * 5 / 2 * (size_t)(Cin > Cout ? Cin : Cout) + 64;
}

int launch_wino4_weights(const float *w, float *U, int G, int Cout, int Cin, hipStream_t st) {
  const long total = (long)G * Cout * Cin;
  long blocks = (total + 255) / 256;
  if (blocks > 4096) blocks = 4096;
  hipLaunchKernelGGL(wino4_weight_kernel, dim3((unsigned)blocks), dim3(256), 0, st, w, U, G, Cout, Cin);
  UOC_LAUNCH_CHECK();
  return UOC_OK;
}

long wino4_elem_blocks(long items) {
  long blocks = (items + 255) / 256;
  const long cap = 16384;
  blocks = blocks < cap ? blocks : cap;
  return (blocks + 7) / 8 * 8;
}

static int launch_wino4_slice(const ConvParams &p0, int Bg, int b0, const float *U, float *ws, hipStream_t st, const W4Tile *tile);

int launch_wino4_conv(const ConvParams &p, const float *U, float *ws, hipStream_t st, const unsigned short *U3, const W4Tile *tile) {
  UOC_REQUIRE(wino4_eligible(p), "winograd F(4x4): layer not eligible");
  UOC_REQUIRE(U && ws && p.in && p.out, "winograd F(4x4): null tensor/weight/workspace pointer");
  const int planes = 36 * p.G;
  UOC_REQUIRE((size_t)planes * p.Cout * p.Cin * 4 < (1ull << 32), "winograd F(4x4): weight planes exceed 4 GB");
  const size_t per_image = (size_t)planes * make_geom4(1, p.H, p.W, p.dil).NT * (p.Cin > p.Cout ? p.Cin : p.Cout) * (U3 ? 6 : 4);
  UOC_REQUIRE(per_image < (1ull << 32), "winograd F(4x4): one image's frequency planes exceed 4 GB");
  static EnvInt limit_mb("UOC_SPLIT_MAX_MB", 0);
  const size_t limit = limit_mb.get() > 0 && ((size_t)limit_mb.get() << 20) > per_image ? (size_t)limit_mb.get() << 20 : (1ull << 32) - 1;
  const int bmax = (int)(limit / per_image);
  if (p.B > bmax) {
    for (int b0 = 0; b0 < p.B; b0 += bmax) {
      ConvParams q = p;
      q.B = p.B - b0 < bmax ? p.B - b0 : bmax;
      if (int rc = U3 ? launch_wino4_slice_split(q, p.B, b0, U3, ws, st, tile) : launch_wino4_slice(q, p.B, b0, U, ws, st, tile)) return rc;
    }
    return UOC_OK;
  }
  return U3 ? launch_wino4_slice_split(p, p.B, 0, U3, ws, st, tile) : launch_wino4_slice(p, p.B, 0, U, ws, st, tile);
}

static int w4_vec() { return 4; }

static int w4_stage_input(const ConvParams &p, const Wino4Geom &geo, float *V, hipStream_t st) {
  const double Mpix = (double)p.B * p.H * p.W;
  const ProfTag tag = {{geo.NT, p.Cin, p.Cout, p.dil}};
  const int vec = w4_vec();
  ProfScope prof(KC_WINO4_INPUT, st, 0.0, 4.0 * p.G * (Mpix * p.Cin + 36.0 * geo.NT * p.Cin), tag);
  const long blocks = wino4_elem_blocks((long)p.G * geo.NT * (p.Cin / vec));
    hipLaunchKernelGGL(wino4_input_kernel<4>, dim3((unsigned)blocks), dim3(256), 0, st, p.in, V, geo, p.G, p.Cin);
  UOC_LAUNCH_CHECK();
  return UOC_OK;
}

static int w4_stage_gemm(const ConvParams &p, const Wino4Geom &geo, const float *U, float *V, float *Mw, hipStream_t st,
                         const W4Tile *tile) {
  const int planes = 36 * p.G;
  const double Mpix = (double)p.B * p.H * p.W;
  const ProfTag tag = {{geo.NT, p.Cin, p.Cout, p.dil}};
  const double gflops = 2.0 * Mpix * p.Cout * p.Cin * 9.0 * p.G;
  const double gbytes = 4.0 * planes * ((double)geo.NT * p.Cin + (double)p.Cout * p.Cin + (double)geo.NT * p.Cout);
  ProfScope prof(KC_WINO4_GEMM, st, gflops, gbytes, tag);
  return launch_wino4_gemm(V, U, Mw, geo.NT, p.Cin, p.Cout, planes, st, tile);
}

int w4_stage_output(const ConvParams &p, const Wino4Geom &geo, const float *Mw, hipStream_t st) {
  const double Mpix = (double)p.B * p.H * p.W;
  const ProfTag tag = {{geo.NT, p.Cin, p.Cout, p.dil}};
  const int vec = w4_vec();
  ProfScope prof(KC_WINO4_OUTPUT, st, 0.0, 4.0 * p.G * (36.0 * geo.NT * p.Cout + Mpix * p.Cout * (p.res ? 2 : 1)), tag);
  const long blocks = wino4_elem_blocks((long)p.G * geo.NT * (p.Cout / vec));
    hipLaunchKernelGGL(wino4_output_kernel<4>, dim3((unsigned)blocks), dim3(256), 0, st, Mw, p.bias, p.res, p.out, geo, p.G, p.Cout, p.relu);
  UOC_LAUNCH_CHECK();
  return UOC_OK;
}

static int launch_wino4_slice(const ConvParams &p0, int Bg, int b0, const float *U, float *ws, hipStream_t st, const W4Tile *tile) {
  ConvParams p = p0;
  const size_t img_in = (size_t)p.H * p.W * p.Cin, img_out = (size_t)p.H * p.W * p.Cout;
  p.in += (size_t)b0 * img_in;
  p.out += (size_t)b0 * img_out;
  if (p.res) p.res += (size_t)b0 * img_out;
  Wino4Geom geo = make_geom4(p.B, p.H, p.W, p.dil);
  geo.Bg = Bg;
  float *V = ws, *Mw = ws + (size_t)36 * p.G * geo.NT * p.Cin;
  if (int rc = w4_stage_input(p, geo, V, st)) return rc;
  if (int rc = w4_stage_gemm(p, geo, U, V, Mw, st, tile)) return rc;
  return w4_stage_output(p, geo, Mw, st);
}

}
```

unseenobjectclustering_amd/csrc/wino4_math.h:

```cpp
#pragma once
#include <hip/hip_runtime.h>

namespace uoc {

struct Wino4Geom {
  int B, H, W, d, TH, TW, NT;
  int Bg;
};

__host__ __device__ inline Wino4Geom make_geom4(int B, int H, int W, int d) {
  Wino4Geom g;
  g.B = B;
  g.H = H;
  g.W = W;
  g.d = d;
  g.TH = ((H + d - 1) / d + 3) / 4;
  g.TW = ((W + d - 1) / d + 3) / 4;
  g.NT = B * d * d * g.TH * g.TW;
  g.Bg = B;
  return g;
}

__host__ __device__ inline void wino4_decode(int tau, const Wino4Geom &g, int &b, int &oy, int &ox) {
  const int tx = tau % g.TW;
  tau /= g.TW;
  const int ty = tau % g.TH;
  tau /= g.TH;
  const int px = tau % g.d;
  tau /= g.d;
  const int py = tau % g.d;
  b = tau / g.d;
  oy = py + 4 * ty * g.d;
  ox = px + 4 * tx * g.d;
}

__host__ __device__ inline float w4_fma(float c, float a, float b) { return fmaf(c, a, b); }
__host__ __device__ inline float w4_add(float a, float b) { return a + b; }
__host__ __device__ inline float w4_sub(float a, float b) { return a - b; }
__host__ __device__ inline float w4_neg(float a) { return -a; }
__host__ __device__ inline float2 w4_fma(float c, float2 a, float2 b) { return make_float2(fmaf(c, a.x, b.x), fmaf(c, a.y, b.y)); }
__host__ __device__ inline float2 w4_add(float2 a, float2 b) { return make_float2(a.x + b.x, a.y + b.y); }
__host__ __device__ inline float2 w4_sub(float2 a, float2 b) { return make_float2(a.x - b.x, a.y - b.y); }
__host__ __device__ inline float2 w4_neg(float2 a) { return make_float2(-a.x, -a.y); }
__host__ __device__ inline float4 w4_fma(float c, float4 a, float4 b) {
  return make_float4(fmaf(c, a.x, b.x), fmaf(c, a.y, b.y), fmaf(c, a.z, b.z), fmaf(c, a.w, b.w));
}
__host__ __device__ inline float4 w4_add(float4 a, float4 b) { return make_float4(a.x + b.x, a.y + b.y, a.z + b.z, a.w + b.w); }
__host__ __device__ inline float4 w4_sub(float4 a, float4 b) { return make_float4(a.x - b.x, a.y - b.y, a.z - b.z, a.w - b.w); }
__host__ __device__ inline float4 w4_neg(float4 a) { return make_float4(-a.x, -a.y, -a.z, -a.w); }

#if defined(__HIP_DEVICE_COMPILE__) && !defined(UOC_W4_NO_NT)
typedef float w4_nv2 __attribute__((ext_vector_type(2)));
typedef float w4_nv4 __attribute__((ext_vector_type(4)));
__device__ inline float w4_nt_load(const float *p) { return __builtin_nontemporal_load(p); }
__device__ inline float2 w4_nt_load(const float2 *p) {
  const w4_nv2 v = __builtin_nontemporal_load(reinterpret_cast<const w4_nv2 *>(p));
  return make_float2(v.x, v.y);
}
__device__ inline float4 w4_nt_load(const float4 *p) {
  const w4_nv4 v = __builtin_nontemporal_load(reinterpret_cast<const w4_nv4 *>(p));
  return make_float4(v.x, v.y, v.z, v.w);
}
__device__ inline void w4_nt_store(float *p, float v) { __builtin_nontemporal_store(v, p); }
__device__ inline void w4_nt_store(float2 *p, float2 v) {
  w4_nv2 n = {v.x, v.y};
  __builtin_nontemporal_store(n, reinterpret_cast<w4_nv2 *>(p));
}
__device__ inline void w4_nt_store(float4 *p, float4 v) {
  w4_nv4 n = {v.x, v.y, v.z, v.w};
  __builtin_nontemporal_store(n, reinterpret_cast<w4_nv4 *>(p));
}
#define W4_STREAM_LOAD(T, ptr) w4_nt_load(reinterpret_cast<const T *>(ptr))
#define W4_STREAM_STORE(T, ptr, val) w4_nt_store(reinterpret_cast<T *>(ptr), (val))
#else
#define W4_STREAM_LOAD(T, ptr) (*reinterpret_cast<const T *>(ptr))
#define W4_STREAM_STORE(T, ptr, val) (*reinterpret_cast<T *>(ptr) = (val))
#endif

template <int VEC> struct W4Vec;
template <> struct W4Vec<1> { typedef float type; };
template <> struct W4Vec<2> { typedef float2 type; };
template <> struct W4Vec<4> { typedef float4 type; };
__host__ __device__ inline void w4_zero(float &v) { v = 0.f; }
__host__ __device__ inline void w4_zero(float2 &v) { v = make_float2(0.f, 0.f); }
__host__ __device__ inline void w4_zero(float4 &v) { v = make_float4(0.f, 0.f, 0.f, 0.f); }
__host__ __device__ inline float w4_relu(float v) { return fmaxf(v, 0.f); }
__host__ __device__ inline float2 w4_relu(float2 v) { return make_float2(fmaxf(v.x, 0.f), fmaxf(v.y, 0.f)); }
__host__ __device__ inline float4 w4_relu(float4 v) { return make_float4(fmaxf(v.x, 0.f), fmaxf(v.y, 0.f), fmaxf(v.z, 0.f), fmaxf(v.w, 0.f)); }

template <typename T>
__host__ __device__ inline void wino4_bt(const T (&i)[6], T (&o)[6]) {
  o[0] = w4_fma(-1.5f, i[3], w4_fma(-2.0f, i[2], w4_fma(1.5f, i[1], w4_add(i[0], i[4]))));
  o[1] = w4_fma(-0.5f, i[3], w4_fma(-2.5f, i[2], w4_sub(i[4], i[1])));
  o[2] = w4_fma(-2.5f, i[3], w4_fma(0.5f, i[2], w4_add(i[4], i[1])));
  o[3] = w4_fma(0.5f, i[3], w4_fma(-0.5f, i[1], w4_sub(i[4], i[2])));
  o[4] = w4_fma(-2.0f, i[3], w4_fma(2.0f, i[1], w4_sub(i[4], i[2])));
  o[5] = w4_fma(-1.5f, i[4], w4_fma(-2.0f, i[3], w4_fma(1.5f, i[2], w4_add(i[1], i[5]))));
}

template <typename T>
__host__ __device__ inline void wino4_at(const T (&m)[6], T (&y)[4]) {
  const T s12 = w4_add(m[1], m[2]), d12 = w4_sub(m[1], m[2]);
  y[0] = w4_add(w4_add(m[0], s12), w4_add(m[3], m[4]));
  y[1] = w4_fma(-0.5f, m[4], w4_fma(2.0f, m[3], d12));
  y[2] = w4_fma(0.25f, m[4], w4_fma(4.0f, m[3], s12));
  y[3] = w4_add(w4_fma(-0.125f, m[4], w4_fma(8.0f, m[3], d12)), m[5]);
}

__host__ __device__ inline void wino4_g(const double (&k)[3], double (&u)[6]) {
  u[0] = k[0];
  u[1] = -(k[0] + k[1] + k[2]) / 3.0;
  u[2] = (k[0] - k[1] + k[2]) / 3.0;
  u[3] = (k[0] + 2.0 * k[1] + 4.0 * k[2]) / 15.0;
  u[4] = (-16.0 * k[0] + 8.0 * k[1] - 4.0 * k[2]) / 15.0;
  u[5] = k[2];
}


__host__ __device__ inline void wino4_weight_body(const float *w, float *U, int G, int Cout, int Cin, int g, int co, int ci) {
  double t[6][3];
  for (int b = 0; b < 3; ++b) {
    const double col[3] = {(double)w[(((size_t)g * 9 + 0 + b) * Cout + co) * Cin + ci],
                           (double)w[(((size_t)g * 9 + 3 + b) * Cout + co) * Cin + ci],
                           (double)w[(((size_t)g * 9 + 6 + b) * Cout + co) * Cin + ci]};
    double u[6];
    wino4_g(col, u);
    for (int i = 0; i < 6; ++i) t[i][b] = u[i];
  }
  const size_t plane = (size_t)Cout * Cin;
  for (int i = 0; i < 6; ++i) {
    double u[6];
    wino4_g(t[i], u);
    for (int j = 0; j < 6; ++j) U[((size_t)g * 36 + 6 * i + j) * plane + (size_t)co * Cin + ci] = (float)u[j];
  }
  (void)G;
}

template <typename T>
__host__ __device__ inline void wino4_input_tile(const T (&d)[6][6], T (&v)[36]) {
  T t[6][6];
#pragma unroll
  for (int j = 0; j < 6; ++j) {
    T col[6], o[6];
#pragma unroll
    for (int i = 0; i < 6; ++i) col[i] = d[i][j];
    wino4_bt(col, o);
#pragma unroll
    for (int i = 0; i < 6; ++i) t[i][j] = o[i];
  }
#pragma unroll
  for (int i = 0; i < 6; ++i) {
    T o[6];
    wino4_bt(t[i], o);
#pragma unroll
    for (int j = 0; j < 6; ++j) v[6 * i + j] = o[j];
  }
}

template <int VEC>
__host__ __device__ inline void wino4_input_body(const float *in, float *V, const Wino4Geom &geo, int C, int g, int tau, int cv) {
  typedef typename W4Vec<VEC>::type T;
  int b, oy, ox;
  wino4_decode(tau, geo, b, oy, ox);
  const float *src = in + (((size_t)g * geo.Bg + b) * geo.H * geo.W) * C + VEC * cv;
  T d[6][6];
#pragma unroll
  for (int j = 0; j < 6; ++j) {
    const int x = ox + (j - 1) * geo.d;
#pragma unroll
    for (int i = 0; i < 6; ++i) {
      const int y = oy + (i - 1) * geo.d;
      const bool ok = (unsigned)y < (unsigned)geo.H && (unsigned)x < (unsigned)geo.W;
      if (ok)
        d[i][j] = *reinterpret_cast<const T *>(src + ((size_t)y * geo.W + x) * C);
      else
        w4_zero(d[i][j]);
    }
  }
  T v[36];
  wino4_input_tile(d, v);
  const size_t plane = (size_t)geo.NT * C;
  float *dst = V + (size_t)g * 36 * plane + (size_t)tau * C + VEC * cv;
#pragma unroll
  for (int k = 0; k < 36; ++k) W4_STREAM_STORE(T, dst + (size_t)k * plane, v[k]);
}

template <typename T>
__host__ __device__ inline void wino4_output_tile(const T (&m)[36], T (&y)[4][4]) {
  T s[4][6];
#pragma unroll
  for (int j = 0; j < 6; ++j) {
    T col[6], o[4];
#pragma unroll
    for (int i = 0; i < 6; ++i) col[i] = m[6 * i + j];
    wino4_at(col, o);
#pragma unroll
    for (int a = 0; a < 4; ++a) s[a][j] = o[a];
  }
#pragma unroll
  for (int a = 0; a < 4; ++a) wino4_at(s[a], y[a]);
}

template <int VEC>
__host__ __device__ inline void wino4_output_body(const float *M, const float *bias, const float *res, float *out,
                                                  const Wino4Geom &geo, int Cout, int relu, int g, int tau, int cv) {
  typedef typename W4Vec<VEC>::type T;
  const size_t plane = (size_t)geo.NT * Cout;
  const float *src = M + (size_t)g * 36 * plane + (size_t)tau * Cout + VEC * cv;
  T m[36];
#pragma unroll
  for (int k = 0; k < 36; ++k) m[k] = W4_STREAM_LOAD(T, src + (size_t)k * plane);
  int b, oy, ox;
  wino4_decode(tau, geo, b, oy, ox);
  const size_t gsz = (size_t)geo.Bg * geo.H * geo.W * Cout;
  const size_t o0 = (size_t)g * gsz + (((size_t)b * geo.H + oy) * geo.W + ox) * Cout + VEC * cv;
  const size_t oy_step = (size_t)geo.d * geo.W * Cout, ox_step = (size_t)geo.d * Cout;
#ifndef W4_OUT_RES_MODE
#define W4_OUT_RES_MODE 2
#endif
  T rv[4][4];
#define W4_LOAD_RES()                                                                        \
  if (res) {                                                                                 \
    _Pragma("unroll") for (int a = 0; a < 4; ++a) _Pragma("unroll") for (int e = 0; e < 4; ++e) { \
      if (oy + a * geo.d < geo.H && ox + e * geo.d < geo.W)                                  \
        rv[a][e] = *reinterpret_cast<const T *>(res + o0 + a * oy_step + e * ox_step);       \
      else                                                                                   \
        w4_zero(rv[a][e]);                                                                   \
    }                                                                                        \
  }
  if (W4_OUT_RES_MODE == 1) { W4_LOAD_RES() }
  T yv[4][4];
  {
    T s[4][6];
#pragma unroll
    for (int j = 0; j < 6; ++j) {
      T col[6], o[4];
#pragma unroll
      for (int i = 0; i < 6; ++i) col[i] = m[6 * i + j];
      wino4_at(col, o);
#pragma unroll
      for (int a = 0; a < 4; ++a) s[a][j] = o[a];
    }
    if (W4_OUT_RES_MODE == 2) { W4_LOAD_RES() }
#pragma unroll
    for (int a = 0; a < 4; ++a) wino4_at(s[a], yv[a]);
  }
#undef W4_LOAD_RES
  T bv;
  if (bias)
    bv = *reinterpret_cast<const T *>(bias + (size_t)g * Cout + VEC * cv);
  else
    w4_zero(bv);
#pragma unroll
  for (int a = 0; a < 4; ++a) {
    const int y = oy + a * geo.d;
    if (y >= geo.H) continue;
#pragma unroll
    for (int e = 0; e < 4; ++e) {
      const int x = ox + e * geo.d;
      if (x >= geo.W) continue;
      T v = w4_add(yv[a][e], bv);
      if (res) v = w4_add(v, W4_OUT_RES_MODE == 0 ? *reinterpret_cast<const T *>(res + o0 + a * oy_step + e * ox_step) : rv[a][e]);
      if (relu) v = w4_relu(v);
      *reinterpret_cast<T *>(out + o0 + a * oy_step + e * ox_step) = v;
    }
  }
}

}
```

Baseline: 176.0 frames/s.

## Skip unused Winograd planes for edge tiles by reordering tiles into classes

Reorders Winograd F(4x4,3x3) tiles into classes by whether each tile's last output row or column falls past the image edge. The input transform, GEMM and output transform then skip the last-row and last-column planes for partial tiles. The GEMM walks per-plane row ranges instead of a fixed tile count. A new DENSE algo id keeps the old full-plane path, which adds index-decode overhead and complexity to the kernels.

```diff
diff --git a/include/uoc_hip.h b/include/uoc_hip.h
--- a/include/uoc_hip.h
+++ b/include/uoc_hip.h
@@ -95,6 +95,7 @@
 #define UOC_CONV_DIRECT 0
 #define UOC_CONV_WINOGRAD4 4
 #define UOC_CONV_WINOGRAD4_BF16X3 5
+#define UOC_CONV_WINOGRAD4_DENSE 6
 int uoc_conv2d_nhwc(const float *d_in, const float *d_w, const float *d_bias, const float *d_res, float *d_out,
                     int G, int B, int H, int W, int Cin, int Cout, int K, int stride, int dil, int pad, int relu,
                     void *stream);
diff --git a/unseenobjectclustering_amd/_native.py b/unseenobjectclustering_amd/_native.py
--- a/unseenobjectclustering_amd/_native.py
+++ b/unseenobjectclustering_amd/_native.py
@@ -267,7 +267,7 @@
     return _lib
 
 
-CONV_DIRECT, CONV_WINOGRAD4, CONV_WINOGRAD4_BF16X3 = 0, 4, 5
+CONV_DIRECT, CONV_WINOGRAD4, CONV_WINOGRAD4_BF16X3, CONV_WINOGRAD4_DENSE = 0, 4, 5, 6
 
 
 def config_fingerprint() -> int:
diff --git a/unseenobjectclustering_amd/csrc/conv.h b/unseenobjectclustering_amd/csrc/conv.h
--- a/unseenobjectclustering_amd/csrc/conv.h
+++ b/unseenobjectclustering_amd/csrc/conv.h
@@ -27,9 +27,12 @@
   int bm, bn;
 };
 int wino4_tile_list(bool split, int *out_pairs, int cap);
-void wino4_tile_choice(bool split, int NT, int Cout, int planes, int *bn, int *bm);
+void wino4_tile_choice(bool split, bool dense, int B, int H, int W, int d, int Cout, int G, int *bn, int *bm);
 int wino4_split_tile_list(int *out_pairs, int cap);
 void wino4_split_tile_choice(int NT, int Cout, int planes, int *bn, int *bm);
+struct Wino4Rows;
+void wino4_pick_tile(const int (*tiles)[2], int n, const Wino4Rows &rows, int Cout, int G, int &bm, int &bn);
+int wino4_plane_grid(const Wino4Rows &rows, int Cout, int G, int bm, int bn);
 void wino4_pick_tile(const int (*tiles)[2], int n, int NT, int Cout, int planes, int &bm, int &bn);
 int wino4_plane_grid(int NT, int Cout, int planes, int bm, int bn);
 
@@ -39,7 +42,7 @@
 int wino4_num_tiles(int B, int H, int W, int d);
 int launch_wino4_weights(const float *w, float *U, int G, int Cout, int Cin, hipStream_t st);
 int launch_wino4_conv(const ConvParams &p, const float *U, float *ws, hipStream_t st, const unsigned short *U3 = nullptr,
-                      const W4Tile *tile = nullptr);
+                      const W4Tile *tile = nullptr, bool dense = false);
 int launch_wino4_split_weights(const float *U, unsigned short *U3, int G, int Cout, int Cin, hipStream_t st);
 int launch_wino4_slice_split(const ConvParams &p0, int Bg, int b0, const unsigned short *U3, float *ws, hipStream_t st,
                              const W4Tile *tile = nullptr);
diff --git a/unseenobjectclustering_amd/csrc/net.hip b/unseenobjectclustering_amd/csrc/net.hip
--- a/unseenobjectclustering_amd/csrc/net.hip
+++ b/unseenobjectclustering_amd/csrc/net.hip
@@ -421,7 +421,7 @@
   const W4Tile *wt = tile ? &w4tile : nullptr;
   static std::mutex mu;
   std::lock_guard<std::mutex> lock(mu);
-  if (algo == UOC_CONV_WINOGRAD4 || algo == UOC_CONV_WINOGRAD4_BF16X3) {
+  if (algo == UOC_CONV_WINOGRAD4 || algo == UOC_CONV_WINOGRAD4_DENSE || algo == UOC_CONV_WINOGRAD4_BF16X3) {
     UOC_REQUIRE(wino4_eligible(p), "conv2d: shape not eligible for Winograd F(4x4,3x3)");
     if (tile) {
       int pairs[2 * 32];
@@ -455,7 +455,7 @@
       if (int rc = launch_wino4_split_weights(U4, U3, G, Cout, Cin, st)) return rc;
       return launch_wino4_conv(p, U4, ws4, st, U3, wt);
     }
-    return launch_wino4_conv(p, U4, ws4, st, nullptr, wt);
+    return launch_wino4_conv(p, U4, ws4, st, nullptr, wt, algo == UOC_CONV_WINOGRAD4_DENSE);
   }
   set_error("conv2d: unknown algorithm %d", algo);
   return UOC_EINVAL;
@@ -478,7 +478,7 @@
 int uoc_conv2d_tile_list(int algo, int32_t *out_pairs, int cap) {
   UOC_REQUIRE(cap >= 0 && (out_pairs || cap == 0), "tile list: null array");
   if (algo == UOC_CONV_DIRECT) return conv_tile_list(out_pairs, cap);
-  if (algo == UOC_CONV_WINOGRAD4 || algo == UOC_CONV_WINOGRAD4_BF16X3)
+  if (algo == UOC_CONV_WINOGRAD4 || algo == UOC_CONV_WINOGRAD4_DENSE || algo == UOC_CONV_WINOGRAD4_BF16X3)
     return wino4_tile_list(algo == UOC_CONV_WINOGRAD4_BF16X3, out_pairs, cap);
   set_error("tile list: unknown algorithm %d", algo);
   return UOC_EINVAL;
@@ -491,10 +491,10 @@
   UOC_REQUIRE(G >= 1 && B >= 1 && H >= 1 && W >= 1 && Cin >= 1 && Cout >= 1 && stride >= 1 && dil >= 1, "tile choice: bad shape");
   const ConvParams p = entry_params(G, B, H, W, Cin, Cout, K, stride, dil, K == 3 ? dil : 0, 0);
   if (algo == UOC_CONV_DIRECT) return conv_tile_choice(p, cfg, bm, family_bm);
-  if (algo == UOC_CONV_WINOGRAD4 || algo == UOC_CONV_WINOGRAD4_BF16X3) {
+  if (algo == UOC_CONV_WINOGRAD4 || algo == UOC_CONV_WINOGRAD4_DENSE || algo == UOC_CONV_WINOGRAD4_BF16X3) {
     UOC_REQUIRE(wino4_eligible(p), "tile choice: shape not eligible for Winograd F(4x4,3x3)");
     int bn_ = 0, bm_ = 0;
-    wino4_tile_choice(algo == UOC_CONV_WINOGRAD4_BF16X3, wino4_num_tiles(B, H, W, dil), Cout, 36 * G, &bn_, &bm_);
+    wino4_tile_choice(algo == UOC_CONV_WINOGRAD4_BF16X3, algo == UOC_CONV_WINOGRAD4_DENSE, B, H, W, dil, Cout, G, &bn_, &bm_);
     *cfg = bn_;
     *bm = bm_;
     return UOC_OK;
diff --git a/unseenobjectclustering_amd/csrc/wino4.hip b/unseenobjectclustering_amd/csrc/wino4.hip
--- a/unseenobjectclustering_amd/csrc/wino4.hip
+++ b/unseenobjectclustering_amd/csrc/wino4.hip
@@ -23,34 +23,36 @@
   }
 }
 
-template <int VEC>
+template <int VEC, int PLAN>
 __global__ __launch_bounds__(256) void wino4_input_kernel(const float *__restrict__ in, float *__restrict__ V,
                                                           Wino4Geom geo, int G, int C) {
   const int CV = C / VEC;
-  const long total = (long)G * geo.NT * CV;
+  const int nwork = PLAN == 1 ? geo.NT : geo.end[3];
+  const long total = (long)G * nwork * CV;
 #ifndef W4_IN_XCD
 #define W4_IN_XCD 1
 #endif
   const long vblock = W4_IN_XCD ? (long)(blockIdx.x & 7) * (gridDim.x >> 3) + (blockIdx.x >> 3) : (long)blockIdx.x;
   for (long idx = vblock * blockDim.x + threadIdx.x; idx < total; idx += (long)gridDim.x * blockDim.x) {
     const int cv = (int)(idx % CV);
-    const int tau = (int)((idx / CV) % geo.NT);
-    const int g = (int)(idx / ((long)CV * geo.NT));
-    wino4_input_body<VEC>(in, V, geo, C, g, tau, cv);
-  }
-}
-
-template <int VEC>
+    const int tau = (int)((idx / CV) % nwork);
+    const int g = (int)(idx / ((long)CV * nwork));
+    wino4_input_body<VEC, PLAN>(in, V, geo, C, g, tau, cv);
+  }
+}
+
+template <int VEC, int PLAN>
 __global__ __launch_bounds__(256, W4_OUT_MIN_BLOCKS) void wino4_output_kernel(const float *__restrict__ M, const float *__restrict__ bias,
                                                            const float *__restrict__ res, float *__restrict__ out,
                                                            Wino4Geom geo, int G, int Cout, int relu) {
   const int CV = Cout / VEC;
-  const long total = (long)G * geo.NT * CV;
+  const int nwork = PLAN == 1 ? geo.NT : geo.end[3];
+  const long total = (long)G * nwork * CV;
   for (long idx = (long)blockIdx.x * blockDim.x + threadIdx.x; idx < total; idx += (long)gridDim.x * blockDim.x) {
     const int cv = (int)(idx % CV);
-    const int tau = (int)((idx / CV) % geo.NT);
-    const int g = (int)(idx / ((long)CV * geo.NT));
-    wino4_output_body<VEC>(M, bias, res, out, geo, Cout, relu, g, tau, cv);
+    const int tau = (int)((idx / CV) % nwork);
+    const int g = (int)(idx / ((long)CV * nwork));
+    wino4_output_body<VEC, PLAN>(M, bias, res, out, geo, Cout, relu, g, tau, cv);
   }
 }
 
@@ -72,7 +74,7 @@
 template <int BM, int BN, bool PAIR, int NW>
 __global__ __launch_bounds__(NW * 64) void wino4_gemm_kernel(const float *__restrict__ V, const float *__restrict__ U,
                                                              float *__restrict__ Mo, int NT, int Cin, int Cout, int planes,
-                                                             int mtiles, int nt_shift) {
+                                                             Wino4Rows rows, int nt_shift) {
   static_assert(NW == 8 || NW == 4, "waves per block");
   constexpr int WAVES_N = NW / 2;
   constexpr int WM = BM / 2, WN = BN / WAVES_N;
@@ -86,8 +88,14 @@
   extern __shared__ __attribute__((aligned(16))) float smem[];
 
   const int ntiles = 1 << nt_shift;
-  const int per_plane = mtiles << nt_shift;
-  const int total = planes * per_plane;
+  const int lo5 = rows.lo5, hi0 = rows.hi[0], hi1 = rows.hi[1], hi2 = rows.hi[2], hi3 = rows.hi[3];
+  const int pp0 = ((hi0 + BM - 1) / BM) << nt_shift, pp1 = ((hi1 + BM - 1) / BM) << nt_shift,
+            pp2 = ((hi2 - lo5 + BM - 1) / BM) << nt_shift, pp3 = ((hi3 - lo5 + BM - 1) / BM) << nt_shift;
+#define W4_KIND_SEL(XI, A, B, C, D) ((XI) < 30 ? ((0x820820820ull >> (XI)) & 1 ? (B) : (A)) : ((XI) == 35 ? (D) : (C)))
+#define W4_PER_PLANE(XI) W4_KIND_SEL(XI, pp0, pp1, pp2, pp3)
+#define W4_NEXT_PLANE(PLANE, XI) { ++PLANE; XI = XI == 35 ? 0 : XI + 1; }
+  const int per_group = 25 * pp0 + 5 * (pp1 + pp2) + pp3;
+  const int total = (planes / 36) * per_group;
   const int S = (total + 7) >> 3;
   const int xcd = blockIdx.x & 7, jloc = blockIdx.x >> 3, nbl = gridDim.x >> 3;
   const int slice_lo = xcd * S, slice_hi = min(total, slice_lo + S);
@@ -120,19 +128,25 @@
     l_c4[j] = 4 * ((lane & 7) ^ ((r >> 1) & 7));
   }
 
-  int iss_plane, iss_rem, iss_cc = 0;
+  int iss_plane, iss_xi = 0, iss_rem, iss_cc = 0;
   {
-    iss_plane = first / per_plane;
-    iss_rem = first - iss_plane * per_plane;
+    const int grp = first / per_group;
+    iss_plane = 36 * grp;
+    iss_rem = first - grp * per_group;
+    for (int pp_ = W4_PER_PLANE(iss_xi); iss_rem >= pp_; pp_ = W4_PER_PLANE(iss_xi)) {
+      iss_rem -= pp_;
+      W4_NEXT_PLANE(iss_plane, iss_xi)
+    }
   }
   unsigned l_voff[NPASS];
   unsigned soff_a, soff_w;
 #define W4_ITEM_SETUP()                                                                                  \
   {                                                                                                      \
     const int mt_ = iss_rem >> nt_shift, nt_ = iss_rem & (ntiles - 1);                                   \
+    const int lo_ = iss_xi < 30 ? 0 : lo5, last_ = W4_KIND_SEL(iss_xi, hi0, hi1, hi2, hi3) - 1;          \
     _Pragma("unroll") for (int j = 0; j < NPASS; ++j) {                                                  \
       if (j < NPA) {                                                                                     \
-        const int tau_ = min(mt_ * BM + l_row[j], NT - 1);                                               \
+        const int tau_ = min(lo_ + mt_ * BM + l_row[j], last_);                                          \
         l_voff[j] = (unsigned)((tau_ * Cin + l_c4[j]) * 4);                                              \
       } else {                                                                                           \
         l_voff[j] = (unsigned)(((nt_ * BN + l_row[j]) * Cin + l_c4[j]) * 4);                             \
@@ -157,9 +171,9 @@
     if (++iss_cc == cpt) {                                                                               \
       iss_cc = 0;                                                                                        \
       iss_rem += nbl;                                                                                    \
-      while (iss_rem >= per_plane) {                                                                     \
-        iss_rem -= per_plane;                                                                            \
-        ++iss_plane;                                                                                     \
+      for (int pp_ = W4_PER_PLANE(iss_xi); iss_rem >= pp_; pp_ = W4_PER_PLANE(iss_xi)) {                 \
+        iss_rem -= pp_;                                                                                  \
+        W4_NEXT_PLANE(iss_plane, iss_xi)                                                                 \
       }                                                                                                  \
       W4_ITEM_SETUP()                                                                                    \
     } else {                                                                                             \
@@ -188,32 +202,33 @@
 #pragma unroll
     for (int i = 0; i < TM; ++i) acc[j][i] = f32x4{0.f, 0.f, 0.f, 0.f};
 
-  int cmp_plane = iss_plane, cmp_rem = iss_rem, cmp_cc = 0;
+  int cmp_plane = iss_plane, cmp_xi = iss_xi, cmp_rem = iss_rem, cmp_cc = 0;
 
   float4 wa0[TN], xb0[TM], wa1[TN], xb1[TM];
   const bool early = NW == 4 || wave < 4;
-  auto epilogue = [&]() {
-    cmp_cc = 0;
-    const int mt = cmp_rem >> nt_shift, nt = cmp_rem & (ntiles - 1);
-    float *dst = Mo + (size_t)cmp_plane * NT * Cout;
-#pragma unroll
-    for (int j = 0; j < TN; ++j) {
-      const int co = nt * BN + wn * WN + 16 * j + 4 * q;
-#pragma unroll
-      for (int i = 0; i < TM; ++i) {
-        const int m = mt * BM + wm * WM + 16 * i + t;
-        if (m < NT)
-          *reinterpret_cast<float4 *>(dst + (size_t)m * Cout + co) =
-              make_float4(acc[j][i][0], acc[j][i][1], acc[j][i][2], acc[j][i][3]);
-        acc[j][i] = f32x4{0.f, 0.f, 0.f, 0.f};
-      }
-    }
-    cmp_rem += nbl;
-    while (cmp_rem >= per_plane) {
-      cmp_rem -= per_plane;
-      ++cmp_plane;
-    }
-  };
+#define W4_EPILOGUE()                                                                                             \
+  {                                                                                                               \
+    cmp_cc = 0;                                                                                                   \
+    const int mt = cmp_rem >> nt_shift, nt = cmp_rem & (ntiles - 1);                                              \
+    const int lo = cmp_xi < 30 ? 0 : lo5, hi = W4_KIND_SEL(cmp_xi, hi0, hi1, hi2, hi3);                           \
+    float *dst = Mo + (size_t)cmp_plane * NT * Cout;                                                              \
+    _Pragma("unroll") for (int j = 0; j < TN; ++j) {                                                              \
+      const int co = nt * BN + wn * WN + 16 * j + 4 * q;                                                          \
+      _Pragma("unroll") for (int i = 0; i < TM; ++i) {                                                            \
+        const int m = lo + mt * BM + wm * WM + 16 * i + t;                                                        \
+         \
+        if (m < hi)                                                                                               \
+          *reinterpret_cast<float4 *>(dst + (size_t)m * Cout + co) =                                              \
+              make_float4(acc[j][i][0], acc[j][i][1], acc[j][i][2], acc[j][i][3]);                                \
+        acc[j][i] = f32x4{0.f, 0.f, 0.f, 0.f};                                                                    \
+      }                                                                                                           \
+    }                                                                                                             \
+    cmp_rem += nbl;                                                                                               \
+    for (int pp = W4_PER_PLANE(cmp_xi); cmp_rem >= pp; pp = W4_PER_PLANE(cmp_xi)) {                               \
+      cmp_rem -= pp;                                                                                              \
+      W4_NEXT_PLANE(cmp_plane, cmp_xi)                                                                            \
+    }                                                                                                             \
+  }
   if constexpr (PAIR) {
     W4_ITEM_SETUP()
     W4_ISSUE(0)
@@ -273,7 +288,7 @@
       __builtin_amdgcn_s_waitcnt(0xC07F);
       __builtin_amdgcn_sched_barrier(0);
       cmp_cc += 2;
-      if (cmp_cc == cpt) epilogue();
+      if (cmp_cc == cpt) W4_EPILOGUE()
     }
     return;
   }
@@ -316,7 +331,7 @@
     __builtin_amdgcn_sched_barrier(0);
     __builtin_amdgcn_s_waitcnt(0xC07F);
     __builtin_amdgcn_sched_barrier(0);
-    if (++cmp_cc == cpt) epilogue();
+    if (++cmp_cc == cpt) W4_EPILOGUE()
     const int tmp = s_cur;
     s_cur = s_nxt;
     s_nxt = s_nn;
@@ -327,12 +342,16 @@
 #undef W4_ADVANCE
 #undef W4_FRAG
 #undef W4_MFMA_E
+#undef W4_EPILOGUE
+#undef W4_KIND_SEL
+#undef W4_PER_PLANE
+#undef W4_NEXT_PLANE
 }
 
 template <int BM, int BN, bool PAIR, int NW>
-static int launch_wino4_gemm_t(const float *V, const float *U, float *Mo, int NT, int Cin, int Cout, int planes, int nblocks,
-                               hipStream_t st) {
-  const int mtiles = (NT + BM - 1) / BM, ntiles = Cout / BN;
+static int launch_wino4_gemm_t(const float *V, const float *U, float *Mo, int NT, const Wino4Rows &rows, int Cin, int Cout,
+                               int planes, int nblocks, hipStream_t st) {
+  const int ntiles = Cout / BN;
   int nt_shift = 0;
   while ((1 << nt_shift) < ntiles) ++nt_shift;
   UOC_REQUIRE((1 << nt_shift) == ntiles, "winograd F(4x4): Cout / %d = %d is not a power of two", BN, ntiles);
@@ -343,13 +362,11 @@
   static DeviceOnce attr_set;
   if (int rc = opt_in_dynamic_lds(reinterpret_cast<const void *>(&wino4_gemm_kernel<BM, BN, PAIR, NW>), lds, attr_set)) return rc;
   hipLaunchKernelGGL((wino4_gemm_kernel<BM, BN, PAIR, NW>), dim3(nblocks), dim3(NW * 64), lds, st, V, U, Mo, NT, Cin, Cout, planes,
-                     mtiles, nt_shift);
+                     rows, nt_shift);
   UOC_LAUNCH_CHECK();
   return UOC_OK;
 }
 
-#define UOC_W4_TILES(X) \
-  X(96, 128) X(128, 128) X(160, 128) X(192, 128) X(96, 64) X(128, 64) X(160, 64) X(192, 64)
 static const int kW4Tiles[][2] = {
 #define X(A, B) {A, B},
     UOC_W4_TILES(X)
@@ -361,13 +378,13 @@
   return ncu / 8 > 0 ? ncu / 8 : 1;
 }
 
-void wino4_pick_tile(const int (*tiles)[2], int n, int NT, int Cout, int planes, int &bm, int &bn) {
+void wino4_pick_tile(const int (*tiles)[2], int n, const Wino4Rows &rows, int Cout, int G, int &bm, int &bn) {
   const int per_xcd = plane_per_xcd();
   double best = -1;
   for (int i = 0; i < n; ++i) {
     const int BM = tiles[i][0], BN = tiles[i][1];
     if (Cout % BN) continue;
-    const long items = (long)planes * ((NT + BM - 1) / BM) * (Cout / BN);
+    const long items = wino4_gemm_items(rows, G, BM, Cout / BN);
     const long S = (items + 7) / 8;
     const long steps = (S + per_xcd - 1) / per_xcd;
     const double cost = (double)steps * BM * BN * (1.0 + 0.05 * (192.0 / BM - 1.0)) * (BN == 64 ? 1.06 : 1.0);
@@ -379,30 +396,39 @@
   }
 }
 
-int wino4_plane_grid(int NT, int Cout, int planes, int bm, int bn) {
+void wino4_pick_tile(const int (*tiles)[2], int n, int NT, int Cout, int planes, int &bm, int &bn) {
+  wino4_pick_tile(tiles, n, wino4_rows_dense(NT), Cout, planes / 36, bm, bn);
+}
+
+int wino4_plane_grid(const Wino4Rows &rows, int Cout, int G, int bm, int bn) {
   const int per_xcd = plane_per_xcd();
-  const long items = (long)planes * ((NT + bm - 1) / bm) * (Cout / bn);
+  const long items = wino4_gemm_items(rows, G, bm, Cout / bn);
   const long S = (items + 7) / 8;
   return 8 * (int)(S < per_xcd ? S : per_xcd);
 }
 
-static int launch_wino4_gemm(const float *V, const float *U, float *Mo, int NT, int Cin, int Cout, int planes, hipStream_t st,
-                             const W4Tile *tile) {
+int wino4_plane_grid(int NT, int Cout, int planes, int bm, int bn) {
+  return wino4_plane_grid(wino4_rows_dense(NT), Cout, planes / 36, bm, bn);
+}
+
+static int launch_wino4_gemm(const float *V, const float *U, float *Mo, int NT, const Wino4Rows &rows, int Cin, int Cout, int G,
+                             hipStream_t st, const W4Tile *tile) {
+  const int planes = 36 * G;
   int bm = 160, bn = Cout % 128 == 0 ? 128 : 64;
   if (tile) {
     bm = tile->bm;
     bn = tile->bn;
     UOC_REQUIRE((bn == 64 || bn == 128) && Cout % bn == 0, "winograd F(4x4): Cout=%d does not admit BN=%d", Cout, bn);
   } else {
-    wino4_pick_tile(kW4Tiles, (int)(sizeof(kW4Tiles) / sizeof(kW4Tiles[0])), NT, Cout, planes, bm, bn);
-  }
-  const int nblocks = wino4_plane_grid(NT, Cout, planes, bm, bn);
+    wino4_pick_tile(kW4Tiles, (int)(sizeof(kW4Tiles) / sizeof(kW4Tiles[0])), rows, Cout, G, bm, bn);
+  }
+  const int nblocks = wino4_plane_grid(rows, Cout, G, bm, bn);
   const int cpt = Cin / W4BK;
   const bool pair = cpt % 2 == 0 && cpt >= 4;
 #define X(A, B)                                                                                                      \
   if (bm == A && bn == B)                                                                                            \
-    return pair ? launch_wino4_gemm_t<A, B, true, 8>(V, U, Mo, NT, Cin, Cout, planes, nblocks, st)                    \
-                : launch_wino4_gemm_t<A, B, false, 8>(V, U, Mo, NT, Cin, Cout, planes, nblocks, st);
+    return pair ? launch_wino4_gemm_t<A, B, true, 8>(V, U, Mo, NT, rows, Cin, Cout, planes, nblocks, st)              \
+                : launch_wino4_gemm_t<A, B, false, 8>(V, U, Mo, NT, rows, Cin, Cout, planes, nblocks, st);
   UOC_W4_TILES(X)
 #undef X
   set_error("winograd F(4x4): no GEMM tile %dx%d", bm, bn);
@@ -419,11 +445,18 @@
   return n;
 }
 
-void wino4_tile_choice(bool split, int NT, int Cout, int planes, int *bn, int *bm) {
-  if (split) return wino4_split_tile_choice(NT, Cout, planes, bn, bm);
+static Wino4Geom w4_plan(int B, int H, int W, int d, bool dense) {
+  if (dense) return make_geom4(B, H, W, d);
+  const Wino4Geom geo = make_geom4_skip(B, H, W, d);
+  return geo.n[W4_FF] == geo.NT ? make_geom4(B, H, W, d) : geo;
+}
+
+void wino4_tile_choice(bool split, bool dense, int B, int H, int W, int d, int Cout, int G, int *bn, int *bm) {
+  const Wino4Geom geo = w4_plan(B, H, W, d, dense || split);
+  if (split) return wino4_split_tile_choice(geo.NT, Cout, 36 * G, bn, bm);
   *bm = 160;
   *bn = Cout % 128 == 0 ? 128 : 64;
-  wino4_pick_tile(kW4Tiles, (int)(sizeof(kW4Tiles) / sizeof(kW4Tiles[0])), NT, Cout, planes, *bm, *bn);
+  wino4_pick_tile(kW4Tiles, (int)(sizeof(kW4Tiles) / sizeof(kW4Tiles[0])), wino4_rows(geo), Cout, G, *bm, *bn);
 }
 
 bool wino4_channels_ok(int Cin, int Cout) {
@@ -459,9 +492,11 @@
   return (blocks + 7) / 8 * 8;
 }
 
-static int launch_wino4_slice(const ConvParams &p0, int Bg, int b0, const float *U, float *ws, hipStream_t st, const W4Tile *tile);
-
-int launch_wino4_conv(const ConvParams &p, const float *U, float *ws, hipStream_t st, const unsigned short *U3, const W4Tile *tile) {
+static int launch_wino4_slice(const ConvParams &p0, int Bg, int b0, const float *U, float *ws, hipStream_t st, const W4Tile *tile,
+                             bool dense);
+
+int launch_wino4_conv(const ConvParams &p, const float *U, float *ws, hipStream_t st, const unsigned short *U3, const W4Tile *tile,
+                      bool dense) {
   UOC_REQUIRE(wino4_eligible(p), "winograd F(4x4): layer not eligible");
   UOC_REQUIRE(U && ws && p.in && p.out, "winograd F(4x4): null tensor/weight/workspace pointer");
   const int planes = 36 * p.G;
@@ -475,11 +510,11 @@
     for (int b0 = 0; b0 < p.B; b0 += bmax) {
       ConvParams q = p;
       q.B = p.B - b0 < bmax ? p.B - b0 : bmax;
-      if (int rc = U3 ? launch_wino4_slice_split(q, p.B, b0, U3, ws, st, tile) : launch_wino4_slice(q, p.B, b0, U, ws, st, tile)) return rc;
+      if (int rc = U3 ? launch_wino4_slice_split(q, p.B, b0, U3, ws, st, tile) : launch_wino4_slice(q, p.B, b0, U, ws, st, tile, dense)) return rc;
     }
     return UOC_OK;
   }
-  return U3 ? launch_wino4_slice_split(p, p.B, 0, U3, ws, st, tile) : launch_wino4_slice(p, p.B, 0, U, ws, st, tile);
+  return U3 ? launch_wino4_slice_split(p, p.B, 0, U3, ws, st, tile) : launch_wino4_slice(p, p.B, 0, U, ws, st, tile, dense);
 }
 
 static int w4_vec() { return 4; }
@@ -488,42 +523,49 @@
   const double Mpix = (double)p.B * p.H * p.W;
   const ProfTag tag = {{geo.NT, p.Cin, p.Cout, p.dil}};
   const int vec = w4_vec();
-  ProfScope prof(KC_WINO4_INPUT, st, 0.0, 4.0 * p.G * (Mpix * p.Cin + 36.0 * geo.NT * p.Cin), tag);
-  const long blocks = wino4_elem_blocks((long)p.G * geo.NT * (p.Cin / vec));
-    hipLaunchKernelGGL(wino4_input_kernel<4>, dim3((unsigned)blocks), dim3(256), 0, st, p.in, V, geo, p.G, p.Cin);
+  ProfScope prof(KC_WINO4_INPUT, st, 0.0, 4.0 * p.G * (Mpix * p.Cin + (double)wino4_plane_pairs(wino4_rows(geo)) * p.Cin), tag);
+  const long blocks = wino4_elem_blocks((long)p.G * geo.end[3] * (p.Cin / vec));
+  if (geo.dense)
+    hipLaunchKernelGGL((wino4_input_kernel<4, 1>), dim3((unsigned)blocks), dim3(256), 0, st, p.in, V, geo, p.G, p.Cin);
+  else
+    hipLaunchKernelGGL((wino4_input_kernel<4, 0>), dim3((unsigned)blocks), dim3(256), 0, st, p.in, V, geo, p.G, p.Cin);
   UOC_LAUNCH_CHECK();
   return UOC_OK;
 }
 
 static int w4_stage_gemm(const ConvParams &p, const Wino4Geom &geo, const float *U, float *V, float *Mw, hipStream_t st,
                          const W4Tile *tile) {
-  const int planes = 36 * p.G;
+  const Wino4Rows rows = wino4_rows(geo);
   const double Mpix = (double)p.B * p.H * p.W;
   const ProfTag tag = {{geo.NT, p.Cin, p.Cout, p.dil}};
   const double gflops = 2.0 * Mpix * p.Cout * p.Cin * 9.0 * p.G;
-  const double gbytes = 4.0 * planes * ((double)geo.NT * p.Cin + (double)p.Cout * p.Cin + (double)geo.NT * p.Cout);
+  const double gbytes = 4.0 * p.G * ((double)wino4_plane_pairs(rows) * (p.Cin + p.Cout) + 36.0 * p.Cout * p.Cin);
   ProfScope prof(KC_WINO4_GEMM, st, gflops, gbytes, tag);
-  return launch_wino4_gemm(V, U, Mw, geo.NT, p.Cin, p.Cout, planes, st, tile);
+  return launch_wino4_gemm(V, U, Mw, geo.NT, rows, p.Cin, p.Cout, p.G, st, tile);
 }
 
 int w4_stage_output(const ConvParams &p, const Wino4Geom &geo, const float *Mw, hipStream_t st) {
   const double Mpix = (double)p.B * p.H * p.W;
   const ProfTag tag = {{geo.NT, p.Cin, p.Cout, p.dil}};
   const int vec = w4_vec();
-  ProfScope prof(KC_WINO4_OUTPUT, st, 0.0, 4.0 * p.G * (36.0 * geo.NT * p.Cout + Mpix * p.Cout * (p.res ? 2 : 1)), tag);
-  const long blocks = wino4_elem_blocks((long)p.G * geo.NT * (p.Cout / vec));
-    hipLaunchKernelGGL(wino4_output_kernel<4>, dim3((unsigned)blocks), dim3(256), 0, st, Mw, p.bias, p.res, p.out, geo, p.G, p.Cout, p.relu);
+  ProfScope prof(KC_WINO4_OUTPUT, st, 0.0, 4.0 * p.G * ((double)wino4_plane_pairs(wino4_rows(geo)) * p.Cout + Mpix * p.Cout * (p.res ? 2 : 1)), tag);
+  const long blocks = wino4_elem_blocks((long)p.G * geo.end[3] * (p.Cout / vec));
+  if (geo.dense)
+    hipLaunchKernelGGL((wino4_output_kernel<4, 1>), dim3((unsigned)blocks), dim3(256), 0, st, Mw, p.bias, p.res, p.out, geo, p.G, p.Cout, p.relu);
+  else
+    hipLaunchKernelGGL((wino4_output_kernel<4, 0>), dim3((unsigned)blocks), dim3(256), 0, st, Mw, p.bias, p.res, p.out, geo, p.G, p.Cout, p.relu);
   UOC_LAUNCH_CHECK();
   return UOC_OK;
 }
 
-static int launch_wino4_slice(const ConvParams &p0, int Bg, int b0, const float *U, float *ws, hipStream_t st, const W4Tile *tile) {
+static int launch_wino4_slice(const ConvParams &p0, int Bg, int b0, const float *U, float *ws, hipStream_t st, const W4Tile *tile,
+                             bool dense) {
   ConvParams p = p0;
   const size_t img_in = (size_t)p.H * p.W * p.Cin, img_out = (size_t)p.H * p.W * p.Cout;
   p.in += (size_t)b0 * img_in;
   p.out += (size_t)b0 * img_out;
   if (p.res) p.res += (size_t)b0 * img_out;
-  Wino4Geom geo = make_geom4(p.B, p.H, p.W, p.dil);
+  Wino4Geom geo = w4_plan(p.B, p.H, p.W, p.dil, dense);
   geo.Bg = Bg;
   float *V = ws, *Mw = ws + (size_t)36 * p.G * geo.NT * p.Cin;
   if (int rc = w4_stage_input(p, geo, V, st)) return rc;
diff --git a/unseenobjectclustering_amd/csrc/wino4_math.h b/unseenobjectclustering_amd/csrc/wino4_math.h
--- a/unseenobjectclustering_amd/csrc/wino4_math.h
+++ b/unseenobjectclustering_amd/csrc/wino4_math.h
@@ -2,10 +2,31 @@
 #include <hip/hip_runtime.h>
 
 namespace uoc {
+
+struct Wino4Axis {
+  int r, f[2], p[2];
+};
+
+__host__ __device__ inline Wino4Axis make_axis4(int n, int d) {
+  Wino4Axis a;
+  a.r = n % d;
+  for (int k = 0; k < 2; ++k) {
+    const int h = n / d + 1 - k;
+    a.f[k] = h / 4;
+    a.p[k] = h % 4 != 0;
+  }
+  return a;
+}
+
+enum { W4_PF = 0, W4_FF = 1, W4_FP = 2, W4_PP = 3, W4_EMPTY = 4 };
 
 struct Wino4Geom {
   int B, H, W, d, TH, TW, NT;
   int Bg;
+  int dense;
+  int n[5];
+  int end[4];
+  Wino4Axis ay, ax;
 };
 
 __host__ __device__ inline Wino4Geom make_geom4(int B, int H, int W, int d) {
@@ -18,10 +39,84 @@
   g.TW = ((W + d - 1) / d + 3) / 4;
   g.NT = B * d * d * g.TH * g.TW;
   g.Bg = B;
+  g.dense = 1;
+  g.ay = make_axis4(H, d);
+  g.ax = make_axis4(W, d);
+  g.n[W4_PF] = g.n[W4_FP] = g.n[W4_PP] = g.n[W4_EMPTY] = 0;
+  g.n[W4_FF] = g.NT;
+  g.end[0] = 0;
+  g.end[1] = g.end[2] = g.end[3] = g.NT;
   return g;
 }
 
-__host__ __device__ inline void wino4_decode(int tau, const Wino4Geom &g, int &b, int &oy, int &ox) {
+__host__ __device__ inline Wino4Geom make_geom4_skip(int B, int H, int W, int d) {
+  Wino4Geom g = make_geom4(B, H, W, d);
+  g.dense = 0;
+  const int yf = g.ay.r * g.ay.f[0] + (d - g.ay.r) * g.ay.f[1], yp = g.ay.r * g.ay.p[0] + (d - g.ay.r) * g.ay.p[1];
+  const int xf = g.ax.r * g.ax.f[0] + (d - g.ax.r) * g.ax.f[1], xp = g.ax.r * g.ax.p[0] + (d - g.ax.r) * g.ax.p[1];
+  g.n[W4_PF] = B * yp * xf;
+  g.n[W4_FF] = B * yf * xf;
+  g.n[W4_FP] = B * yf * xp;
+  g.n[W4_PP] = B * yp * xp;
+  g.end[0] = g.n[0];
+  for (int c = 1; c < 4; ++c) g.end[c] = g.end[c - 1] + g.n[c];
+  g.n[W4_EMPTY] = g.NT - g.end[3];
+  return g;
+}
+
+__host__ __device__ inline void wino4_tile_class(int tau, const Wino4Geom &g, bool &row4, bool &col4) {
+  row4 = g.dense || (tau >= g.end[0] && tau < g.end[2]);
+  col4 = g.dense || tau < g.end[1];
+}
+
+struct Wino4Rows {
+  int lo5;
+  int hi[4];
+};
+
+__host__ __device__ inline Wino4Rows wino4_rows(const Wino4Geom &g) {
+  Wino4Rows r;
+  r.lo5 = g.end[0];
+  r.hi[0] = g.end[3];
+  r.hi[1] = g.end[1];
+  r.hi[2] = g.end[2];
+  r.hi[3] = g.end[1];
+  return r;
+}
+__host__ __device__ inline Wino4Rows wino4_rows_dense(int NT) {
+  Wino4Rows r;
+  r.lo5 = 0;
+  r.hi[0] = r.hi[1] = r.hi[2] = r.hi[3] = NT;
+  return r;
+}
+__host__ __device__ inline int wino4_plane_kind(int xi) { return (xi >= 30 ? 2 : 0) | (int)((0x820820820ull >> xi) & 1); }
+__host__ __device__ inline void wino4_plane_rows(const Wino4Rows &r, int xi, int &lo, int &hi) {
+  const int kind = wino4_plane_kind(xi);
+  lo = kind >= 2 ? r.lo5 : 0;
+  hi = kind == 0 ? r.hi[0] : kind == 1 ? r.hi[1] : kind == 2 ? r.hi[2] : r.hi[3];
+}
+__host__ __device__ inline long wino4_plane_pairs(const Wino4Rows &r) {
+  return 25l * r.hi[0] + 5l * r.hi[1] + 5l * (r.hi[2] - r.lo5) + (r.hi[3] - r.lo5);
+}
+#define UOC_W4_TILES(X) \
+  X(96, 128) X(128, 128) X(160, 128) X(192, 128) X(96, 64) X(128, 64) X(160, 64) X(192, 64)
+inline long wino4_gemm_items(const Wino4Rows &r, int G, int BM, int ntiles) {
+  const long m0 = (r.hi[0] + BM - 1) / BM, m1 = (r.hi[1] + BM - 1) / BM, m2 = (r.hi[2] - r.lo5 + BM - 1) / BM,
+             m3 = (r.hi[3] - r.lo5 + BM - 1) / BM;
+  return (long)G * ntiles * (25 * m0 + 5 * m1 + 5 * m2 + m3);
+}
+
+__host__ __device__ inline void w4_axis_decode(const Wino4Axis &a, int kind, int T, int k, int &phase, int &t) {
+  const int nl = kind == 0 ? a.f[0] : kind == 1 ? a.p[0] : T - a.f[0] - a.p[0], ol = kind == 0 ? 0 : kind == 1 ? a.f[0] : a.f[0] + a.p[0];
+  const int ns = kind == 0 ? a.f[1] : kind == 1 ? a.p[1] : T - a.f[1] - a.p[1], os = kind == 0 ? 0 : kind == 1 ? a.f[1] : a.f[1] + a.p[1];
+  const bool lng = k < a.r * nl;
+  const int n = lng ? nl : ns, kk = lng ? k : k - a.r * nl;
+  const int q = kk / n;
+  phase = (lng ? 0 : a.r) + q;
+  t = (lng ? ol : os) + kk - q * n;
+}
+
+__host__ __device__ inline void wino4_decode_dense(int tau, const Wino4Geom &g, int &b, int &oy, int &ox) {
   const int tx = tau % g.TW;
   tau /= g.TW;
   const int ty = tau % g.TH;
@@ -34,6 +129,58 @@
   ox = px + 4 * tx * g.d;
 }
 
+__host__ __device__ inline void wino4_decode_skip(int tau, const Wino4Geom &g, int &b, int &oy, int &ox) {
+  const int d = g.d;
+  const int yf = g.ay.r * g.ay.f[0] + (d - g.ay.r) * g.ay.f[1], yp = g.ay.r * g.ay.p[0] + (d - g.ay.r) * g.ay.p[1];
+  const int xf = g.ax.r * g.ax.f[0] + (d - g.ax.r) * g.ax.f[1], xp = g.ax.r * g.ax.p[0] + (d - g.ax.r) * g.ax.p[1];
+  int ky, kx, ny, nx, py, ty, px, tx;
+#if !defined(__HIP_DEVICE_COMPILE__)
+  if (tau >= g.end[3]) {
+    tau -= g.end[3];
+    const int ye = d * g.TH - yf - yp, xall = d * g.TW;
+    if (tau < g.B * ye * xall) {
+      const int xk = tau % xall;
+      tau /= xall;
+      w4_axis_decode(g.ay, 2, g.TH, tau % ye, py, ty);
+      b = tau / ye;
+      oy = py + 4 * ty * d;
+      ox = xk / g.TW + 4 * (xk % g.TW) * d;
+      return;
+    }
+    tau -= g.B * ye * xall;
+    ky = -1;
+    kx = 2;
+    ny = yf + yp;
+    nx = d * g.TW - xf - xp;
+  } else
+#endif
+  {
+    ky = tau < g.end[0] || tau >= g.end[2];
+    kx = tau >= g.end[1];
+    tau -= tau < g.end[0] ? 0 : tau < g.end[1] ? g.end[0] : tau < g.end[2] ? g.end[1] : g.end[2];
+    ny = ky ? yp : yf;
+    nx = kx ? xp : xf;
+  }
+  const int t = tau / nx, xk = tau - t * nx;
+  b = t / ny;
+  int yk = t - b * ny;
+  if (ky < 0) {
+    ky = yk >= yf;
+    if (ky) yk -= yf;
+  }
+  w4_axis_decode(g.ay, ky, g.TH, yk, py, ty);
+  w4_axis_decode(g.ax, kx, g.TW, xk, px, tx);
+  oy = py + 4 * ty * d;
+  ox = px + 4 * tx * d;
+}
+
+__host__ __device__ inline void wino4_decode(int tau, const Wino4Geom &g, int &b, int &oy, int &ox) {
+  if (g.dense)
+    wino4_decode_dense(tau, g, b, oy, ox);
+  else
+    wino4_decode_skip(tau, g, b, oy, ox);
+}
+
 __host__ __device__ inline float w4_fma(float c, float a, float b) { return fmaf(c, a, b); }
 __host__ __device__ inline float w4_add(float a, float b) { return a + b; }
 __host__ __device__ inline float w4_sub(float a, float b) { return a - b; }
@@ -157,11 +304,19 @@
   }
 }
 
-template <int VEC>
+template <int VEC, int PLAN = -1>
 __host__ __device__ inline void wino4_input_body(const float *in, float *V, const Wino4Geom &geo, int C, int g, int tau, int cv) {
   typedef typename W4Vec<VEC>::type T;
+  const bool dense = PLAN < 0 ? geo.dense != 0 : PLAN == 1;
+  if (!dense && tau >= geo.end[3]) return;
   int b, oy, ox;
-  wino4_decode(tau, geo, b, oy, ox);
+  bool row4 = true, col4 = true;
+  if (dense) {
+    wino4_decode_dense(tau, geo, b, oy, ox);
+  } else {
+    wino4_decode_skip(tau, geo, b, oy, ox);
+    wino4_tile_class(tau, geo, row4, col4);
+  }
   const float *src = in + (((size_t)g * geo.Bg + b) * geo.H * geo.W) * C + VEC * cv;
   T d[6][6];
 #pragma unroll
@@ -182,7 +337,8 @@
   const size_t plane = (size_t)geo.NT * C;
   float *dst = V + (size_t)g * 36 * plane + (size_t)tau * C + VEC * cv;
 #pragma unroll
-  for (int k = 0; k < 36; ++k) W4_STREAM_STORE(T, dst + (size_t)k * plane, v[k]);
+  for (int k = 0; k < 36; ++k)
+    if ((k < 30 || row4) && (k % 6 != 5 || col4)) W4_STREAM_STORE(T, dst + (size_t)k * plane, v[k]);
 }
 
 template <typename T>
@@ -201,17 +357,30 @@
   for (int a = 0; a < 4; ++a) wino4_at(s[a], y[a]);
 }
 
-template <int VEC>
+template <int VEC, int PLAN = -1>
 __host__ __device__ inline void wino4_output_body(const float *M, const float *bias, const float *res, float *out,
                                                   const Wino4Geom &geo, int Cout, int relu, int g, int tau, int cv) {
   typedef typename W4Vec<VEC>::type T;
+  const bool dense = PLAN < 0 ? geo.dense != 0 : PLAN == 1;
   const size_t plane = (size_t)geo.NT * Cout;
   const float *src = M + (size_t)g * 36 * plane + (size_t)tau * Cout + VEC * cv;
+  if (!dense && tau >= geo.end[3]) return;
+  int b, oy, ox;
+  bool row4 = true, col4 = true;
+  if (!dense) {
+    wino4_decode_skip(tau, geo, b, oy, ox);
+    row4 = oy + 3 * geo.d < geo.H;
+    col4 = ox + 3 * geo.d < geo.W;
+  }
   T m[36];
 #pragma unroll
-  for (int k = 0; k < 36; ++k) m[k] = W4_STREAM_LOAD(T, src + (size_t)k * plane);
-  int b, oy, ox;
-  wino4_decode(tau, geo, b, oy, ox);
+  for (int k = 0; k < 36; ++k) {
+    if ((k < 30 || row4) && (k % 6 != 5 || col4))
+      m[k] = W4_STREAM_LOAD(T, src + (size_t)k * plane);
+    else
+      w4_zero(m[k]);
+  }
+  if (dense) wino4_decode_dense(tau, geo, b, oy, ox);
   const size_t gsz = (size_t)geo.Bg * geo.H * geo.W * Cout;
   const size_t o0 = (size_t)g * gsz + (((size_t)b * geo.H + oy) * geo.W + ox) * Cout + VEC * cv;
   const size_t oy_step = (size_t)geo.d * geo.W * Cout, ox_step = (size_t)geo.d * Cout;
```

Measured after the change: 180.0 frames/s (median of 6 runs). 1.02x the previous value.
